# The-Learning-And-Vision-Atelier-LAVA/BUFFER

Measured on AMD Instinct MI355X. Metric: registration pairs/sec, higher is better.
Workload: dtype f32

## Files before the change

buffer_amd/_lib.py:

```python
import ctypes as C
import os

_HERE = os.path.dirname(os.path.abspath(__file__))
LIB_PATH = os.environ.get("BUF_LIB_PATH") or os.path.join(_HERE, "libbuffer_hip.so")

BUF_OK = 0


class BufferHipError(RuntimeError):
    pass


class buf_grid_t(C.Structure):
    _fields_ = [
        ("ws", C.c_void_p), ("ws_bytes", C.c_size_t),
        ("ns", C.c_int), ("nb", C.c_int),
        ("cells_per_elem", C.c_int64),
        ("radius", C.c_float),
        ("supports", C.c_void_p),
        ("desc", C.c_void_p), ("s_off", C.c_void_p), ("table", C.c_void_p),
        ("sorted", C.c_void_p), ("order", C.c_void_p), ("scan_tmp", C.c_void_p),
    ]


class buf_voxel_map_t(C.Structure):
    _fields_ = [
        ("buf", C.c_void_p), ("buf_bytes", C.c_size_t),
        ("nclouds", C.c_int), ("nrows", C.c_int), ("n", C.c_int),
        ("max_cells", C.c_int64),
        ("voxel", C.c_double), ("epsilon", C.c_double),
        ("clouds", C.c_void_p), ("table", C.c_void_p), ("rows", C.c_void_p), ("keys", C.c_void_p), ("row_off", C.c_void_p),
    ]


_lib = None

_vp, _i, _f, _i64, _sz = C.c_void_p, C.c_int, C.c_float, C.c_int64, C.c_size_t

_SIGNATURES = {
    "buf_last_error": (C.c_char_p, []),
    "buf_version": (_i, []),
    "buf_device_count": (_i, []),
    "buf_timing_enable": (None, [_i]),
    "buf_timing_collect": (C.c_longlong, [C.POINTER(C.c_double), C.POINTER(C.c_double)]),
    "buf_timing_collect_kernel": (C.c_longlong, [_i, C.POINTER(C.c_double), C.POINTER(C.c_double)]),
    "buf_grid_default_cells": (_i64, [_i, _i]),
    "buf_grid_ws_bytes": (_sz, [_i, _i, _i64]),
    "buf_grid_cell_dims": (_i, [C.POINTER(C.c_double), _f, _i64, C.POINTER(C.c_double), C.POINTER(C.c_int)]),
    "buf_grid_build": (_i, [C.POINTER(buf_grid_t), _vp, _i, _vp, _i, _f, _i64, _vp, _sz, _vp]),
    "buf_grid_query": (_i, [C.POINTER(buf_grid_t), _vp, _i, _vp, _vp, _f, _i, _vp, _vp, _vp, _vp, _vp]),
    "buf_radius_neighbors": (_i, [_vp, _i, _vp, _i, _vp, _vp, _i, _f, _i, _vp, _vp, _vp, _vp, _sz, _vp]),
    "buf_grid_subsample_ws_bytes": (_sz, [_i, _i, _i64, _i]),
    "buf_grid_subsample_batch": (_i, [_vp, _i, _vp, _i, _f, _i, _vp, _i, _vp, _vp, _vp, _vp, _i64, _vp, _sz, _vp]),
    "buf_fps_ws_bytes": (_sz, [_i, _i]),
    "buf_fps": (_i, [_vp, _i, _i, _i, _vp, _vp, _sz, _vp]),
    "buf_gather": (_i, [_vp, _vp, _i, _i, _i, _i, _vp, _vp]),
    "buf_group": (_i, [_vp, _vp, _i, _i, _i, _i, _i, _vp, _vp]),
    "buf_ball_query": (_i, [_vp, _vp, _i, _i, _i, _f, _i, _vp, _vp]),
    "buf_three_nn": (_i, [_vp, _vp, _i, _i, _i, _vp, _vp, _vp]),
    "buf_select_patches": (_i, [_vp, _vp, _i, _i, _f, _i, _vp, _vp]),
    "buf_select_patches_batched_ws_bytes": (_sz, [_i, _i]),
    "buf_select_patches_batched": (_i, [_vp, _vp, _i, _vp, _i, _f, _i, _vp, _vp, _sz, _vp]),
    "buf_permute_clouds": (_i, [_vp, _vp, _vp, _i, _vp, _vp]),
    "buf_compact_ws_bytes": (_sz, [_i]),
    "buf_compact_greater": (_i, [_vp, _i, _i, _f, _vp, _vp, _vp, _sz, _vp]),
    "buf_knn_ws_bytes": (_sz, [_i, _i, _i]),
    "buf_knn1_ws_bytes": (_sz, [_i, _i, _i]),
    "buf_knn": (_i, [_vp, _vp, _i, _i, _i, _i, _i, _vp, _vp, _vp, _sz, _vp]),
    "buf_fps_ragged": (_i, [_vp, _vp, _i, _i, _vp, _vp, _sz, _vp]),
    "buf_svd3x3_batched": (_i, [_vp, _i, _vp, _vp, _vp, _vp]),
    "buf_vn_gather_block": (_i, [_vp, _vp, _vp, _vp, _i, _i, _i, _i, _i, _i, _f, _vp, _vp, _vp, _vp, _f, _vp, _vp]),
    "buf_vn_gather_pre_supported": (_i, [_i, _i, _i]),
    "buf_vn_gather_pre_ws_bytes": (_sz, [_i, _i]),
    "buf_vn_gather_block_pre": (_i, [_vp, _vp, _vp, _vp, _i, _i, _i, _i, _i, _f, _vp, _vp, _vp, _vp, _f, _vp, _vp, _sz, _vp]),
    "buf_vn_pointwise": (_i, [_vp, _vp, _i, _i, _i, _vp, _i, _i, _i, _vp, _vp, _vp, _vp, _f, _vp, _vp, _vp]),
    "buf_gather_max": (_i, [_vp, _vp, _i, _i, _i, _i, _vp, _vp]),
    "buf_vn_std": (_i, [_vp, _vp, _i, _i, _vp, _vp]),
    "buf_score_head_ws_bytes": (_sz, [_i, _i]),
    "buf_score_head": (_i, [_vp, _i, _vp, _i, _vp, _vp, _vp, _vp, _f, _vp, _vp, _vp, _vp, _f, _vp, _vp, _vp, _vp, _vp, _i, _vp, _vp, _i, _f,
                            _vp, _vp, _sz, _vp]),
    "buf_patch_voxelize_ws_bytes": (_sz, [_i]),
    "buf_patch_voxelize": (_i, [_vp, _vp, _i, _i, _f, _vp, _i, _i, _vp, _f, _i, _vp, _vp, _vp, _vp, _vp, _vp, _vp,
                                _vp, _vp, _sz, _vp]),
    "buf_cylindrical_net_wg": (_i, [_vp, _i, _vp, _vp, _vp, _vp, _vp, _vp, _vp]),
    "buf_cylindrical_net_wg_form": (_i, [_vp, _i, _vp, _vp, _vp, _vp, _vp, _i, _vp, _vp]),
    "buf_cylindrical_net_wg_all": (_i, [_vp, _i, _vp, _vp, _vp, _vp, _vp, _vp, _vp, _vp]),
    "buf_cylindrical_net_wg_all_flags": (_i, [_vp, _vp, _vp, _vp]),
    "buf_cylindrical_net_w25": (_i, [_vp, _i, _vp, _vp, _vp, _vp, _vp, _vp, _vp, _vp, _vp]),
    "buf_cylindrical_net_w25_flags": (_i, [_vp, _vp, _vp, _vp, _vp]),
    "buf_cylindrical_net_split_safe_w25": (_i, [_vp, _i, _vp, _vp, _vp, _vp, _vp, _vp, _vp, _vp, _vp, _vp, _vp, _vp, _vp, _vp]),
    "buf_winograd_f25_tile_weights": (_i, [_vp, _i, _i, _vp]),
    "buf_cylindrical_net_wg_supports": (_i, [_vp, _vp]),
    "buf_cylindrical_net_wg_flags": (_i, [_vp, _vp, _vp]),
    "buf_cylindrical_net_split_safe": (_i, [_vp, _i, _vp, _vp, _vp, _vp, _vp, _vp, _vp, _vp, _vp, _vp, _vp, _vp]),
    "buf_cylindrical_net_split_safe_form": (_i, [_vp, _i, _vp, _vp, _vp, _vp, _vp, _vp, _i, _vp, _vp, _vp, _vp, _vp, _vp]),
    "buf_cost_volume_net_split_safe": (_i, [_vp, _vp, _i, _vp, _vp, _i, _vp, _vp, _vp, _vp, _vp, _vp, _vp, _vp]),
    "buf_cylindrical_net_split_safe_all": (_i, [_vp, _i, _vp, _vp, _vp, _vp, _vp, _vp, _vp, _vp, _vp, _vp, _vp, _vp, _vp]),
    "buf_cylindrical_net_split": (_i, [_vp, _i, _vp, _vp, _vp, _vp, _vp, _vp, _vp, _vp]),
    "buf_cylindrical_net_split_head": (_i, [_vp, _i, _vp, _vp, _vp, _vp, _vp, _vp, _vp, _vp, _vp, _vp]),
    "buf_split_gemm_count": (C.c_longlong, [_i, _i, _i, _i]),
    "buf_split_tile_gemm": (_i, [_vp, _i, _i, _i, _i, _vp]),
    "buf_cost_volume_net_split": (_i, [_vp, _vp, _i, _vp, _vp, _vp, _vp, _vp]),
    "buf_cost_volume_net_split_gather": (_i, [_vp, _i, _vp, _vp, _i, _vp, _vp, _vp, _vp, _vp]),
    "buf_split_filter_count": (C.c_longlong, [_i, _i]),
    "buf_split_tile_filters": (_i, [_vp, _i, _i, _vp]),
    "buf_winograd_tile_weights": (_i, [_vp, _i, _i, _vp]),
    "buf_winograd_f24_tile_weights": (_i, [_vp, _i, _i, _vp]),
    "buf_winograd_group": (_i, [_i, _i]),
    "buf_cost_winograd_group": (_i, [_i]),
    "buf_winograd_tile_filters": (_i, [_vp, _i, _i, _i, _i, _vp]),
    "buf_voxel_downsample_ws_bytes": (_sz, [_i, _i64]),
    "buf_voxel_downsample": (_i, [_vp, _vp, _i, _i, C.c_double, _vp, _vp, _vp, _i64, _vp, _sz, _vp]),
    "buf_voxel_downsample_batch_ws_bytes": (_sz, [_i, _i, _i64]),
    "buf_voxel_downsample_batch": (_i, [_vp, _i, _i, _vp, _i, C.c_double, _vp, _vp, _i64, _vp, _sz, _vp]),
    "buf_knn_normals": (_i, [_vp, _i, _vp, _i, _vp, _i, _i, _vp, _i, _vp, _vp, _vp]),
    "buf_icp_ws_bytes": (_sz, [_i, _i, _i, _i]),
    "buf_icp_batched": (_i, [_vp, _vp, _vp, _vp, _vp, _i, _i, _f, _vp, _i, C.c_double, C.c_double, _vp, _vp, _vp, _vp, _vp,
                             _vp, _sz, _vp]),
    "buf_gicp_batched": (_i, [_vp, _vp, _vp, _vp, _vp, _vp, _i, _f, C.c_double, _vp, _i, C.c_double, C.c_double, _vp, _vp, _vp, _vp,
                              _vp, _vp, _sz, _vp]),
    "buf_pair_stats_ws_bytes": (_sz, [_i, _i, _i, _i, _i64]),
    "buf_pair_stats": (_i, [_vp, _vp, _i, _vp, _vp, _i, _vp, _f, _i64, _vp, _vp, _vp, _vp, _sz, _vp]),
    "buf_pose_graph_ws_bytes": (_sz, [_i, _i, _i, _i]),
    "buf_pose_graph_optimize": (_i, [_vp, _vp, _i, _vp, _vp, _vp, _vp, _vp, _vp, _vp, _vp, _i, C.c_double, C.c_double, C.c_double,
                                     _vp, _vp, _vp, _vp, _vp, _sz, _vp]),
    "buf_fpfh_ws_bytes": (_sz, [_i]),
    "buf_fpfh": (_i, [_vp, _vp, _i, _vp, _i, _i, _vp, _vp, _vp, _sz, _vp]),
    "buf_iss_keypoints": (_i, [_vp, _i, _vp, _i, _vp, _i, _i, C.c_double, C.c_double, _i, _vp, _vp, _vp, _vp]),
    "buf_feature_match_ws_bytes": (_sz, [C.c_longlong, C.c_longlong, _i]),
    "buf_feature_match": (_i, [_vp, _vp, _vp, _vp, _i, _i, _i, _f, _vp, _vp, _vp, _vp, _vp, _sz, _vp]),
    "buf_fgr_ws_bytes": (_sz, [_i, _i, _i]),
    "buf_fgr_batched": (_i, [_vp, _vp, _vp, _vp, _vp, _vp, _i, _vp, C.c_double, _i, _i, C.c_double, C.c_double, _i, C.c_double, _i, _i,
                             _vp, _vp, _vp, _vp, _vp, _sz, _vp]),
    "buf_sc2_ws_bytes": (_sz, [_vp, _i, _i]),
    "buf_sc2_batched": (_i, [_vp, _vp, _vp, _vp, _vp, _vp, _i, C.c_double, C.c_double, C.c_double, _i, _i, C.c_double, _i, _i,
                             _vp, _vp, _vp, _vp, _vp, _vp, _vp, _vp, _sz, _vp]),
    "buf_clique_ws_bytes": (_sz, [_vp, _i, _i, _i]),
    "buf_clique_batched": (_i, [_vp, _vp, _vp, _vp, _vp, _vp, _i, C.c_double, C.c_double, C.c_double, C.c_double, _i, _i, C.c_double, _i,
                                _i, _vp, _vp, _vp, _vp, _vp, _vp, _vp, _vp, _vp, _vp, _vp, _sz, _vp]),
    "buf_voxel_map_bytes": (_sz, [_i, _i, _i64]),
    "buf_voxel_map_ws_bytes": (_sz, [_i, _i, _i64]),
    "buf_voxel_map_build": (_i, [C.POINTER(buf_voxel_map_t), _vp, _vp, _vp, _i, C.c_double, C.c_double, _i64, _vp, _sz, _vp, _sz, _vp]),
    "buf_voxel_map_export": (_i, [C.POINTER(buf_voxel_map_t), _i, _vp, _vp, _vp, _vp, _vp, _vp]),
    "buf_vgicp_ws_bytes": (_sz, [_i, _i]),
    "buf_vgicp_batched": (_i, [C.POINTER(buf_voxel_map_t), _vp, _vp, _vp, _vp, _i, _i, _vp, _i, C.c_double, C.c_double, _vp, _vp, _vp,
                               _vp, _vp, _vp, _sz, _vp]),
    "buf_match_metrics":(_i, [_vp, _vp, _vp, _i, _i, _vp, _vp, _f, _f, _f, _vp, _vp, _vp]),
    "buf_row_linear": (_i, [_vp, _i, _i, _i, _vp, _vp, _i, _vp, _vp]),
    "buf_segment_instance_norm_ws_bytes": (_sz, [_i, _i]),
    "buf_segment_instance_norm": (_i, [_vp, _i, _i, _vp, _i, _f, _vp, _vp, _sz, _vp]),
    "buf_descriptor_head": (_i, [_vp, _i, _vp, _vp, _vp, _vp]),
    "buf_cost_volume_net": (_i, [_vp, _vp, _i, _vp, _vp, _vp, _vp]),
    "buf_cost_volume_net_gather": (_i, [_vp, _i, _vp, _vp, _i, _vp, _vp, _vp, _vp]),
    "buf_cost_volume_net_w24": (_i, [_vp, _vp, _i, _vp, _vp, _vp, _vp, _vp]),
    "buf_cost_volume_net_w24_gather": (_i, [_vp, _i, _vp, _vp, _i, _vp, _vp, _vp, _vp, _vp]),
    "buf_cost_volume_net_split_safe_w24": (_i, [_vp, _vp, _i, _vp, _vp, _i, _vp, _vp, _vp, _vp, _vp, _vp, _vp, _vp, _vp]),
    "buf_cost_volume_net_w24b": (_i, [_vp, _vp, _i, _vp, _vp, _vp, _vp, _vp]),
    "buf_cost_volume_net_w24b_gather": (_i, [_vp, _i, _vp, _vp, _i, _vp, _vp, _vp, _vp, _vp]),
    "buf_cost_volume_net_split_safe_w24b": (_i, [_vp, _vp, _i, _vp, _vp, _i, _vp, _vp, _vp, _vp, _vp, _vp, _vp, _vp, _vp]),
    "buf_hypotheses_score": (_i, [_vp, _vp, _vp, _vp, _vp, _i, _i, _f, _vp, _vp, _vp, _vp, _vp, _vp]),
    "buf_ransac_ws_bytes": (_sz, [_i]),
    "buf_ransac_kabsch": (_i, [_vp, _vp, _vp, _i, _i, C.c_uint64, _f, _f, _vp, _vp, _vp, _sz, _vp]),
    "buf_ransac_masked_ws_bytes": (_sz, [_i, _i]),
    "buf_ransac_kabsch_masked": (_i, [_vp, _vp, _vp, _i, _i, C.c_uint64, _f, _f, _vp, _vp, _vp, _sz, _vp]),
    "buf_post_refine": (_i, [_vp, _vp, _vp, _i, _f, _i, _vp, _vp, _vp]),
    "buf_recover_poses_ws_bytes": (_sz, [_i, _i, _i]),
    "buf_recover_poses_batched": (_i, [_vp, _vp, _vp, _vp, _vp, _vp, _i, _vp, _i, _f, _i, _f, _f, _f, _i, _vp, _vp, _sz, _vp]),
}


def exported_symbols():
    return sorted(_SIGNATURES)


def lib():
    global _lib
    if _lib is None:
        if not os.path.exists(LIB_PATH):
            raise BufferHipError(
                f"{LIB_PATH} is missing: build it with `python -m buffer_amd.build` "
                "(hipcc --offload-arch=gfx950). buffer_amd has no CPU fallback.")
        import torch
        l = C.CDLL(LIB_PATH)
        for name, (res, args) in _SIGNATURES.items():
            fn = getattr(l, name)
            fn.restype = res
            fn.argtypes = args
        _lib = l
    return _lib


def check(rc, what=""):
    if rc != BUF_OK:
        msg = lib().buf_last_error().decode(errors="replace")
        raise BufferHipError(f"{what} failed ({rc}): {msg}")
```

buffer_amd/csrc/buffer_hip.hip:

```cpp
#include <stdlib.h>
#include "core.hip"
#include "radius.hip"
#include "icp.hip"
#include "pairstats.hip"
#include "posegraph.hip"
#include "metrics.hip"
#include "subsample.hip"
#include "pointops.hip"
#include "vn.hip"
#include "voxelize.hip"
#include "registration.hip"
#include "convnet.hip"
#include "convnet_h3.hip"
#include "costnet_h3.hip"
#include "preprocess.hip"
#include "convnet_wg.hip"
#include "convnet_w24.hip"
#include "convnet_w24k.hip"
#include "convnet_w24p.hip"
#include "convnet_w24a.hip"
#include "convnet_w25.hip"
#include "costnet.hip"
#include "costnet_w24.hip"
#include "costnet_w24b.hip"
#include "cnn_launch.hip"
#include "split_safe.hip"
#include "fpfh.hip"
#include "iss.hip"
#include "match.hip"
#include "fgr.hip"
#include "sc2.hip"
#include "clique.hip"
#include "vgicp.hip"
```

buffer_amd/csrc/cnn_launch.hip:

```cpp
#include "common.h"

#define WG_F24_FLAG BUF_CYL_F24
#define BUF_CYL_FORM_LIBRARY BUF_CYL_FORM_PASS_SPLIT
static inline bool wg_f24_flagged(int relu) { return relu >= 2; }

typedef void (*CylKernelFn)(const float*, CylWgParams, float*);
struct CylKernel { CylKernelFn plain, rerun; LdsGrant grant, grant_rerun; };
static CylKernel cyl_wg = { k_cyl_net_wg, k_cyl_net_wg_rerun }, cyl_w24 = { k_cyl_net_w24, k_cyl_net_w24_rerun },
                 cyl_w24k = { k_cyl_net_w24k, k_cyl_net_w24k_rerun }, cyl_w24p = { k_cyl_net_w24p, k_cyl_net_w24p_rerun },
                 cyl_w24a = { k_cyl_net_w24a, k_cyl_net_w24a_rerun }, cyl_w25 = { k_cyl_net_w25, k_cyl_net_w25_rerun };

static CylKernel& cyl_kernel_for(const int* relu, int form, bool sets24, bool sets25)
{
    if (sets25) return cyl_w25;
    if (sets24) return cyl_w24a;
    bool flagged = false, ksplit = false;
    for (int l = 0; l < WG_LAYERS; l++) {
        flagged |= wg_f24_flagged(relu[l]);
        ksplit |= (relu[l] & BUF_CYL_F24K) != 0;
    }
    if (!flagged) return cyl_wg;
    if (!ksplit) return cyl_w24;
    if (form == BUF_CYL_FORM_DEFAULT) form = BUF_CYL_FORM_LIBRARY;
    return form == BUF_CYL_FORM_PASS_SPLIT ? cyl_w24p : cyl_w24k;
}

static int wg_check_widths(const int* cin, const int* cout, bool follow = true)
{
    for (int l = 0; l < WG_LAYERS; l++) {
        const int ci = cin[l], co = cout[l];
        BUF_REQUIRE(ci > 0 && ci % 16 == 0 && ci <= WG_MAXC && (co == 32 || co == 64 || co == 128), BUF_EINVAL,
                    "buf_cylindrical_net_wg: layer %d has unsupported widths %d -> %d", l, ci, co);
        BUF_REQUIRE(co != 128 || ci % 32 == 0, BUF_EINVAL,
                    "buf_cylindrical_net_wg: layer %d has unsupported widths %d -> %d (128 output channels need Cin %% 32 == 0)", l, ci, co);
        BUF_REQUIRE(co != 32 || (ci % 32 == 0 && ci <= 64), BUF_EINVAL,
                    "buf_cylindrical_net_wg: layer %d has unsupported widths %d -> %d (32 output channels need Cin = 32 or 64)", l, ci, co);
        BUF_REQUIRE(l == 0 || ci == cout[l - 1], BUF_EINVAL, "buf_cylindrical_net_wg: layer %d width mismatch", l);
        BUF_REQUIRE(!follow || l == 0 || cout[l - 1] != 32 || co == 32, BUF_EINVAL,
                    "buf_cylindrical_net_wg: layer %d has unsupported widths %d -> %d (only 32-output layers may follow a 32-output layer)", l, ci, co);
    }
    BUF_REQUIRE(cout[WG_LAYERS - 1] == 32, BUF_EINVAL, "buf_cylindrical_net_wg: the last layer must have 32 channels");
    return BUF_OK;
}

static int w24_check_flags(const int* cin, const int* cout, const int* relu)
{
    for (int l = 0; l < WG_LAYERS; l++) {
        BUF_REQUIRE(relu[l] >= 0 && relu[l] <= (BUF_CYL_F24K | WG_F24_FLAG | 1), BUF_EINVAL,
                    "buf_cylindrical_net_wg: layer %d has the relu word %d (bit 0: ReLU, bits 1 and 2: the F(2x4) flags, nothing above)", l, relu[l]);
        BUF_REQUIRE(!(relu[l] & BUF_CYL_F24K) || (cout[l] == 64 && cin[l] % 64 == 0), BUF_EINVAL,
                    "buf_cylindrical_net_wg: the K-split F(2x4) flag (bit 2) goes only on layers with 64 output channels and Cin %% 64 == 0 "
                    "(layer %d: %d -> %d, flags %d)", l, cin[l], cout[l], relu[l]);
        BUF_REQUIRE(((relu[l] & WG_F24_FLAG) != 0) == (cout[l] == 128), BUF_EINVAL,
                    "buf_cylindrical_net_wg: the F(2x4) flag goes on every layer with 128 output channels and on no other (layer %d: %d -> %d, flags %d)",
                    l, cin[l], cout[l], relu[l]);
    }
    return BUF_OK;
}

static int cyl_check(const int* cin, const int* cout, const int* relu, const float* const* wt24_host, const float* const* wt25_host, const char* who)
{
    if (!wt24_host && !wt25_host) {
        if (int rc = wg_check_widths(cin, cout)) return rc;
        for (int l = 0; l < WG_LAYERS; l++)
            if (wg_f24_flagged(relu[l])) return w24_check_flags(cin, cout, relu);
        return BUF_OK;
    }
    for (int l = 0; wt25_host && l < WG_LAYERS; l++)
        BUF_REQUIRE(!wt25_host[l] || ((cout[l] == 64 || cout[l] == 32) && cin[l] > 0 && cin[l] % 16 == 0), BUF_EINVAL,
                    "%s: layer %d (%d -> %d) takes no F(2x5) set (64 or 32 output channels, Cin %% 16 == 0)", who, l, cin[l], cout[l]);
    if (int rc = wg_check_widths(cin, cout, false)) return rc;
    if (int rc = w24_check_flags(cin, cout, relu)) return rc;
    bool f22_ran = false;
    int f22_layer = -1;
    for (int l = 0; l < WG_LAYERS; l++) {
        const bool own24 = wt24_host && wt24_host[l], own25 = wt25_host && wt25_host[l];
        BUF_REQUIRE(!own24 || (!(relu[l] & (WG_F24_FLAG | W24K_FLAG)) && (cout[l] == 64 || cout[l] == 32)), BUF_EINVAL,
                    "%s: layer %d (%d -> %d, flags %d) takes no F(2x4) set of its own (64 or 32 output channels, no F(2x4) flag)",
                    who, l, cin[l], cout[l], relu[l]);
        BUF_REQUIRE(!f22_ran || cout[l] == 32, BUF_EINVAL,
                    "%s: layer %d has unsupported widths %d -> %d (once a 32-output layer in the F(2x2) form has run, layer %d here, "
                    "only 32-output layers may follow)", who, l, cin[l], cout[l], f22_layer);
        if (cout[l] == 32 && !own24 && !own25 && !f22_ran) { f22_ran = true; f22_layer = l; }
    }
    return BUF_OK;
}

extern "C" int buf_cylindrical_net_wg_supports(const int* cin_host, const int* cout_host)
{
    BUF_REQUIRE(cin_host && cout_host, BUF_EINVAL, "buf_cylindrical_net_wg_supports: null argument");
    return wg_check_widths(cin_host, cout_host);
}

extern "C" int buf_cylindrical_net_wg_flags(const int* cin_host, const int* cout_host, const int* relu_host)
{
    BUF_REQUIRE(cin_host && cout_host && relu_host, BUF_EINVAL, "buf_cylindrical_net_wg_flags: null argument");
    return cyl_check(cin_host, cout_host, relu_host, nullptr, nullptr, "buf_cylindrical_net_wg");
}

extern "C" int buf_cylindrical_net_wg_all_flags(const int* cin_host, const int* cout_host, const int* relu_host, const float* const* wt24_host)
{
    BUF_REQUIRE(cin_host && cout_host && relu_host && wt24_host, BUF_EINVAL, "buf_cylindrical_net_wg_all_flags: null argument");
    return cyl_check(cin_host, cout_host, relu_host, wt24_host, nullptr, "buf_cylindrical_net_wg_all");
}

extern "C" int buf_cylindrical_net_w25_flags(const int* cin_host, const int* cout_host, const int* relu_host, const float* const* wt24_host,
                                             const float* const* wt25_host)
{
    BUF_REQUIRE(cin_host && cout_host && relu_host && wt24_host && wt25_host, BUF_EINVAL, "buf_cylindrical_net_w25_flags: null argument");
    return cyl_check(cin_host, cout_host, relu_host, wt24_host, wt25_host, "buf_cylindrical_net_w25");
}

static int cyl_prepare(const float* const* wt_host, const float* const* bias_host, const int* cin_host, const int* cout_host, const int* relu_host,
                       const float* const* wt24_host, const float* const* wt25_host, int form, const char* who, CylWgParams& P, CylKernel*& K)
{
    BUF_REQUIRE(wt_host && bias_host && cin_host && cout_host && relu_host, BUF_EINVAL, "%s: null argument", who);
    for (int l = 0; l < WG_LAYERS; l++) {
        P.wt[l] = wt_host[l]; P.bias[l] = bias_host[l];
        P.cin[l] = cin_host[l]; P.cout[l] = cout_host[l]; P.relu[l] = relu_host[l];
        BUF_REQUIRE(P.wt[l] && P.bias[l], BUF_EINVAL, "%s: null weights for layer %d", who, l);
    }
    if (int rc = cyl_check(P.cin, P.cout, P.relu, wt24_host, wt25_host, who)) return rc;
    P.only_if = nullptr;
    K = &cyl_kernel_for(P.relu, form, wt24_host != nullptr, wt25_host != nullptr);
    if (K == &cyl_wg) return BUF_OK;
    for (int l = 0; l < WG_LAYERS; l++) {
        if (wt25_host && wt25_host[l]) { P.wt[l] = wt25_host[l]; P.relu[l] = (P.relu[l] & 1) | W25_FLAG; }
        else if (P.relu[l] & WG_F24_FLAG) P.wt[l] += W24_SET_F22(P.cin[l]);
        else if (P.relu[l] & W24K_FLAG) P.wt[l] += WG_BLOCKS * P.cout[l] * P.cin[l];
        else if (wt24_host && wt24_host[l]) { P.wt[l] = wt24_host[l]; P.relu[l] |= W24K_FLAG; }
        P.relu[l] &= ~WG_F24_FLAG;
    }
    return BUF_OK;
}

#ifdef WG_STAMP
static int wg_stamp_report(const CylWgParams& P, int npatch, void* stream)
{
    BUF_CHECK_HIP(hipStreamSynchronize((hipStream_t)stream));
    long long* h = (long long*)malloc((size_t)npatch * (4 * 20 + 4) * sizeof(long long));
    BUF_CHECK_HIP(hipMemcpy(h, P.stamps, (size_t)npatch * (4 * 20 + 4) * sizeof(long long), hipMemcpyDeviceToHost));
    double comp[WG_LAYERS][4] = {}, wait[WG_LAYERS][4] = {}, tot = 0, pre = 0; long n = 0;
    for (int b = npatch / 2; b < npatch; b++, n++)
        for (int w = 0; w < 4; w++) {
            const long long* q = h + ((size_t)b * 4 + w) * 20;
            for (int l = 0; l < WG_LAYERS; l++) { comp[l][w] += (double)(q[2 * l + 1] - q[2 * l]); wait[l][w] += (double)(q[2 * l + 2] - q[2 * l + 1]); }
            if (w == 0) { tot += (double)(q[2 * WG_LAYERS] - q[0]); pre += (double)(q[0] - q[17]); }
        }
    if (n && npatch >= 1024) {
        double dc = 0, dr = 0;
        for (int b = npatch / 2; b < npatch; b++) { const long long* q = h + (size_t)npatch * 80 + (size_t)b * 4; dc += (double)(q[2] - q[0]); dr += (double)(q[3] - q[1]); }
        fprintf(stderr, "  WG_STAMP in-kernel clock: %.0f shader cycles per workgroup over %.0f ticks of the 100 MHz counter -> %.3f GHz\n", dc / n, dr / n, dc / dr * 0.1);
        fprintf(stderr, "WG_STAMP: %ld workgroups, layers total %.0f cycles per patch, input phase %.0f\n", n, tot / n, pre / n);
        for (int l = 0; l < WG_LAYERS; l++) {
            const double mf = 38.0 * (P.cin[l] / 4) * (P.cout[l] / 16) / 4;
            fprintf(stderr, "  layer %d %3d->%3d: MFMAs/wave %5.0f | to barrier %7.0f %7.0f %7.0f %7.0f | wait %6.0f %6.0f %6.0f %6.0f | cycles per MFMA slot %.1f\n",
                    l, P.cin[l], P.cout[l], mf, comp[l][0] / n, comp[l][1] / n, comp[l][2] / n, comp[l][3] / n, wait[l][0] / n, wait[l][1] / n,
                    wait[l][2] / n, wait[l][3] / n, (comp[l][0] + wait[l][0]) / n / (2 * mf));
        }
    }
    free(h); (void)hipFree(P.stamps);
    return BUF_OK;
}
#endif

static int cyl_launch(CylKernel& K, const float* x, int npatch, CylWgParams P, float* y, void* stream)
{
    const size_t lds = sizeof(float) * WG_BUF;
    if (int rc = P.only_if ? grant_dynamic_lds((const void*)K.rerun, lds, K.grant_rerun) : grant_dynamic_lds((const void*)K.plain, lds, K.grant)) return rc;
    double macs = 0;
    for (int l = 0; l < WG_LAYERS; l++) macs += 9.0 * P.cin[l] * P.cout[l];
    TimedSpan span;
    bool timed = !P.only_if && timing_begin((hipStream_t)stream, &span, 2.0 * 140 * macs * npatch, BUF_TIMED_CYL_NET);
#ifdef WG_STAMP
    if (&K == &cyl_wg) BUF_CHECK_HIP(hipMalloc(&P.stamps, (size_t)npatch * (4 * 20 + 4) * sizeof(long long)));
#endif
    const CylKernelFn kernel = P.only_if ? K.rerun : K.plain;
    kernel<<<npatch, WG_THREADS, lds, (hipStream_t)stream>>>(x, P, y);
    if (timed) timing_end((hipStream_t)stream, &span);
    BUF_LAUNCH_CHECK();
#ifdef WG_STAMP
    if (&K == &cyl_wg) return wg_stamp_report(P, npatch, stream);
#endif
    return BUF_OK;
}

extern "C" int buf_cylindrical_net_wg_form(const float* x, int npatch, const float* const* wt_host, const float* const* bias_host,
                                           const int* cin_host, const int* cout_host, const int* relu_host, int form, float* y, void* stream)
{
    BUF_REQUIRE(npatch >= 0, BUF_EINVAL, "buf_cylindrical_net_wg: npatch=%d", npatch);
    BUF_REQUIRE(form >= BUF_CYL_FORM_DEFAULT && form <= BUF_CYL_FORM_PASS_SPLIT, BUF_EINVAL,
                "buf_cylindrical_net_wg: form=%d (-1: the library's default, 0: K split, 1: pass split)", form);
    if (npatch == 0) return BUF_OK;
    BUF_REQUIRE(x && y, BUF_EINVAL, "buf_cylindrical_net_wg: null argument");
    CylWgParams P;
    CylKernel* K;
    if (int rc = cyl_prepare(wt_host, bias_host, cin_host, cout_host, relu_host, nullptr, nullptr, form, "buf_cylindrical_net_wg", P, K)) return rc;
    return cyl_launch(*K, x, npatch, P, y, stream);
}

extern "C" int buf_cylindrical_net_wg(const float* x, int npatch, const float* const* wt_host, const float* const* bias_host,
                                      const int* cin_host, const int* cout_host, const int* relu_host, float* y, void* stream)
{
    return buf_cylindrical_net_wg_form(x, npatch, wt_host, bias_host, cin_host, cout_host, relu_host, BUF_CYL_FORM_DEFAULT, y, stream);
}

static int cyl_net_own_sets(const char* who, const float* x, int npatch, const float* const* wt_host, const float* const* bias_host, const int* cin_host,
                            const int* cout_host, const int* relu_host, const float* const* wt24_host, const float* const* wt25_host, bool w25, float* y,
                            void* stream)
{
    BUF_REQUIRE(npatch >= 0, BUF_EINVAL, "%s: npatch=%d", who, npatch);
    if (npatch == 0) return BUF_OK;
    BUF_REQUIRE(x && y && wt24_host && (wt25_host || !w25), BUF_EINVAL, "%s: null argument", who);
    CylWgParams P;
    CylKernel* K;
    if (int rc = cyl_prepare(wt_host, bias_host, cin_host, cout_host, relu_host, wt24_host, wt25_host, BUF_CYL_FORM_DEFAULT, who, P, K)) return rc;
    return cyl_launch(*K, x, npatch, P, y, stream);
}

extern "C" int buf_cylindrical_net_wg_all(const float* x, int npatch, const float* const* wt_host, const float* const* bias_host, const int* cin_host,
                                          const int* cout_host, const int* relu_host, const float* const* wt24_host, float* y, void* stream)
{
    return cyl_net_own_sets("buf_cylindrical_net_wg_all", x, npatch, wt_host, bias_host, cin_host, cout_host, relu_host, wt24_host, nullptr, false, y, stream);
}

extern "C" int buf_cylindrical_net_w25(const float* x, int npatch, const float* const* wt_host, const float* const* bias_host, const int* cin_host,
                                       const int* cout_host, const int* relu_host, const float* const* wt24_host, const float* const* wt25_host, float* y,
                                       void* stream)
{
    return cyl_net_own_sets("buf_cylindrical_net_w25", x, npatch, wt_host, bias_host, cin_host, cout_host, relu_host, wt24_host, wt25_host, true, y, stream);
}

template <typename Q>
struct CostKernel { void (*plain)(const float*, const float*, Q, float*); void (*rerun)(const float*, const float*, Q, float*); const char* name; LdsGrant grant, grant_rerun; };
static CostKernel<CostNetParams> cost_f22 = { k_cost_net, k_cost_net_rerun, "k_cost_net" };
static CostKernel<CostNetW24Params> cost_w24 = { k_cost_net_w24, k_cost_net_w24_rerun, "k_cost_net_w24" };
static CostKernel<CostNetW24BParams> cost_w24b = { k_cost_net_w24b, k_cost_net_w24b_rerun, "k_cost_net_w24b" };

static CostNetParams& cost_net_base(CostNetParams& P) { return P; }
template <typename Q> static CostNetParams& cost_net_base(Q& q) { return q.P; }
static void cost_net_sets(CostNetParams&, const float* const*) {}
template <typename Q> static void cost_net_sets(Q& q, const float* const* f24_host)
{
    for (size_t i = 0; i < sizeof(q.f24) / sizeof(q.f24[0]); i++) q.f24[i] = f24_host[i];
}

template <typename Q>
static int cost_net_prepare(Q& q, const float* const* wt_host, const float* const* bias_host, const float* const* f24_host, const long long* s_rows,
                            const long long* t_rows, int ele_n, const int* only_if, const char* who)
{
    CostNetParams& P = cost_net_base(q);
    for (int l = 0; l < CV_LAYERS; l++) {
        P.wt[l] = wt_host[l]; P.bias[l] = bias_host[l];
        BUF_REQUIRE(P.wt[l] && P.bias[l], BUF_EINVAL, "%s: null weights for layer %d", who, l);
    }
    P.s_rows = s_rows; P.t_rows = t_rows;
    P.chan_floats = s_rows ? ele_n * 20 : 100;
    P.row_floats = 32 * P.chan_floats;
    P.skip_floats = s_rows ? 20 : 0;
    P.only_if = only_if;
    cost_net_sets(q, f24_host);
    return BUF_OK;
}

static const double cost_net_macs_per_match =
    60.0 * 480 * 32 + 54.0 * 288 * 32 + 16.0 * 64 * 96 * 64 +
    16.0 * (49.0 * 64 * 64 + 36.0 * 64 * 128 + 25.0 * 128 * 128 + 16.0 * 128 * 64) +
    36.0 * 576 * 64 + 16.0 * 576 * 32 + 4.0 * 288 * 32 + 1.0 * 128 * 20;

#ifdef CV_STAMP
static int cv_stamp_begin(int m, long long** stamps)
{
    BUF_CHECK_HIP(hipMalloc(stamps, (size_t)m * 16 * sizeof(long long)));
    BUF_CHECK_HIP(hipMemcpyToSymbol(HIP_SYMBOL(cv_stamp_ptr), stamps, sizeof(*stamps)));
    return BUF_OK;
}
static int cv_stamp_end(int m, long long* stamps, void* stream, const char* kernel)
{
    if (m >= 2048) {
        BUF_CHECK_HIP(hipStreamSynchronize((hipStream_t)stream));
        long long* h = (long long*)malloc((size_t)m * 16 * sizeof(long long));
        BUF_CHECK_HIP(hipMemcpy(h, stamps, (size_t)m * 16 * sizeof(long long), hipMemcpyDeviceToHost));
        static const char* name[8] = { "A.1 (layer 0 maps)", "A.2 (layer 1)", "layer 2", "layer 3", "layer 4", "layer 5", "layer 6", "layers 7-9" };
        double d[8] = {};
        for (int b = m / 2; b < m; b++)
            for (int i = 0; i < 8; i++) d[i] += (double)(h[(size_t)b * 16 + i + 1] - h[(size_t)b * 16 + i]);
        for (int i = 0; i < 8; i++) fprintf(stderr, "  CV_STAMP %s %-20s %8.0f cycles per match\n", kernel, name[i], d[i] / (m - m / 2));
        free(h);
    }
    (void)hipFree(stamps);
    return BUF_OK;
}
#endif

template <typename Q>
static int cost_net_launch(CostKernel<Q>& K, const float* s_eq, const float* t_eq, int m, Q q, float* ind_out, void* stream)
{
    const bool rerun = cost_net_base(q).only_if != nullptr;
    size_t lds = sizeof(float) * CV_BUF;
    if (int rc = rerun ? grant_dynamic_lds((const void*)K.rerun, lds, K.grant_rerun) : grant_dynamic_lds((const void*)K.plain, lds, K.grant)) return rc;
    TimedSpan span;
    bool timed = !rerun && timing_begin((hipStream_t)stream, &span, 2.0 * cost_net_macs_per_match * m, BUF_TIMED_COST_NET);
#ifdef CV_STAMP
    long long* stamps = nullptr;
    if (int rc = cv_stamp_begin(m, &stamps)) return rc;
#endif
    const auto kernel = rerun ? K.rerun : K.plain;
    kernel<<<m, CV_THREADS, lds, (hipStream_t)stream>>>(s_eq, t_eq, q, ind_out);
    if (timed) timing_end((hipStream_t)stream, &span);
    BUF_LAUNCH_CHECK();
#ifdef CV_STAMP
    if (int rc = cv_stamp_end(m, stamps, stream, K.name)) return rc;
#endif
    return BUF_OK;
}

template <typename Q>
static int cost_net_run(const char* who, CostKernel<Q>& K, bool gathered, const float* s_eq, const float* t_eq, int ele_n, const long long* s_rows,
                        const long long* t_rows, int m, const float* const* wt_host, const float* const* bias_host, const float* const* f24_host,
                        float* ind_out, void* stream)
{
    if (gathered) BUF_REQUIRE(m >= 0 && ele_n == 7, BUF_EINVAL, "%s: m=%d ele_n=%d (the kernel is built for ele_n = 7)", who, m, ele_n);
    else BUF_REQUIRE(m >= 0, BUF_EINVAL, "%s: m=%d", who, m);
    if (m == 0) return BUF_OK;
    BUF_REQUIRE(s_eq && t_eq && (!gathered || (s_rows && t_rows)) && wt_host && bias_host && (f24_host || std::is_same<Q, CostNetParams>::value) && ind_out,
                BUF_EINVAL, "%s: null argument", who);
    Q q;
    if (int rc = cost_net_prepare(q, wt_host, bias_host, f24_host, s_rows, t_rows, ele_n, nullptr, who)) return rc;
    return cost_net_launch(K, s_eq, t_eq, m, q, ind_out, stream);
}

extern "C" int buf_cost_volume_net(const float* s_eq, const float* t_eq, int m, const float* const* wt_host,
                                   const float* const* bias_host, float* ind_out, void* stream)
{
    return cost_net_run("buf_cost_volume_net", cost_f22, false, s_eq, t_eq, 7, nullptr, nullptr, m, wt_host, bias_host, nullptr, ind_out, stream);
}

extern "C" int buf_cost_volume_net_gather(const float* equi, int ele_n, const long long* s_rows, const long long* t_rows, int m,
                                          const float* const* wt_host, const float* const* bias_host, float* ind_out, void* stream)
{
    return cost_net_run("buf_cost_volume_net_gather", cost_f22, true, equi, equi, ele_n, s_rows, t_rows, m, wt_host, bias_host, nullptr, ind_out, stream);
}

extern "C" int buf_cost_volume_net_w24(const float* s_eq, const float* t_eq, int m, const float* const* wt_host, const float* const* bias_host,
                                       const float* const* f24_host, float* ind_out, void* stream)
{
    return cost_net_run("buf_cost_volume_net_w24", cost_w24, false, s_eq, t_eq, 7, nullptr, nullptr, m, wt_host, bias_host, f24_host, ind_out, stream);
}

extern "C" int buf_cost_volume_net_w24_gather(const float* equi, int ele_n, const long long* s_rows, const long long* t_rows, int m,
                                              const float* const* wt_host, const float* const* bias_host, const float* const* f24_host,
                                              float* ind_out, void* stream)
{
    return cost_net_run("buf_cost_volume_net_w24_gather", cost_w24, true, equi, equi, ele_n, s_rows, t_rows, m, wt_host, bias_host, f24_host, ind_out, stream);
}

extern "C" int buf_cost_volume_net_w24b(const float* s_eq, const float* t_eq, int m, const float* const* wt_host, const float* const* bias_host,
                                        const float* const* f24_host, float* ind_out, void* stream)
{
    return cost_net_run("buf_cost_volume_net_w24b", cost_w24b, false, s_eq, t_eq, 7, nullptr, nullptr, m, wt_host, bias_host, f24_host, ind_out, stream);
}

extern "C" int buf_cost_volume_net_w24b_gather(const float* equi, int ele_n, const long long* s_rows, const long long* t_rows, int m,
                                               const float* const* wt_host, const float* const* bias_host, const float* const* f24_host,
                                               float* ind_out, void* stream)
{
    return cost_net_run("buf_cost_volume_net_w24b_gather", cost_w24b, true, equi, equi, ele_n, s_rows, t_rows, m, wt_host, bias_host, f24_host, ind_out, stream);
}
```

buffer_amd/csrc/convnet_wg.hip:

```cpp
#include "common.h"
#include <type_traits>

#define WG_CS 160
#define WG_ROW 22
#define WG_ZERO 154
#define WG_MAXC 128
#define WG_LAYERS 8
#define WG_THREADS 256
#define WG_BUF (WG_MAXC * WG_CS)
#define WG_KSTEP (16 * WG_CS)
#define WG_BLOCKS 16

typedef float wgf4 __attribute__((ext_vector_type(4)));
typedef float wgf2 __attribute__((ext_vector_type(2)));
typedef const __attribute__((address_space(3))) wgf2* wg_lds_f2;

struct CylWgParams {
    const float* wt[WG_LAYERS];
    const float* bias[WG_LAYERS];
    int cin[WG_LAYERS], cout[WG_LAYERS], relu[WG_LAYERS];
    const int* only_if;
#ifdef WG_STAMP
    long long* stamps;
#endif
};
#ifdef WG_STAMP
#define WG_STAMP_AT(SLOT) if ((threadIdx.x & 63) == 0) P.stamps[((size_t)blockIdx.x * 4 + w) * 20 + (SLOT)] = __builtin_amdgcn_s_memtime();
#else
#define WG_STAMP_AT(SLOT)
#endif

__device__ __forceinline__ bool wg_tile(int t, int idx, int& ty, int& tx)
{
    if (t == 0) { const bool a = idx < 10; ty = a ? 0 : 1; tx = a ? idx : idx - 6; return true; }
    if (t == 1) { const bool a = idx < 10, b = idx < 14; ty = a ? 2 : (b ? 1 : 3); tx = a ? idx : (b ? idx - 10 : idx - 6); return true; }
    ty = 3; tx = 0;
    return false;
}

__device__ __forceinline__ unsigned wg_row_addr(unsigned act_addr, int t, int a, int li, int lk)
{
    if (t == 2) return act_addr + 4u * (unsigned)(lk * WG_CS + (a < 2 ? (5 + a) * WG_ROW + li : WG_ZERO));
    int ty, tx;
    const bool ok = wg_tile(t, li, ty, tx);
    const int row = 2 * ty - 1 + a;
    return act_addr + 4u * (unsigned)(lk * WG_CS + ((ok && row >= 0 && row <= 6) ? row * WG_ROW + 2 * tx : WG_ZERO));
}

__device__ __forceinline__ float wg_add(float a, float b) { float r; asm("v_add_f32 %0, %1, %2" : "=v"(r) : "v"(a), "v"(b)); return r; }
__device__ __forceinline__ float wg_sub(float a, float b) { float r; asm("v_sub_f32 %0, %1, %2" : "=v"(r) : "v"(a), "v"(b)); return r; }

__host__ __device__ constexpr int wg_a1(int I) { return I == 0 ? 0 : 1; }
__host__ __device__ constexpr int wg_a2(int I) { return I == 3 ? 3 : 2; }

__host__ __device__ constexpr bool wg_chains(int I) { return I >= 0 && I < 3; }

#define WG_LOAD2(DST, A0, A1_, OFS)                                                                       \
    {                                                                                                     \
        DST[0] = *(wg_lds_f2)(size_t)((A0) + (OFS));                                                      \
        asm volatile("" : "+v"(A0));                                                                      \
        DST[1] = *(wg_lds_f2)(size_t)((A0) + (OFS) + 8);                                                  \
        asm volatile("" : "+v"(A0));                                                                      \
        DST[2] = *(wg_lds_f2)(size_t)((A1_) + (OFS));                                                     \
        asm volatile("" : "+v"(A1_));                                                                     \
        DST[3] = *(wg_lds_f2)(size_t)((A1_) + (OFS) + 8);                                                 \
        asm volatile("" : "+v"(A1_));                                                                     \
    }


typedef unsigned wgu4 __attribute__((ext_vector_type(4)));
__device__ __forceinline__ __amdgpu_buffer_rsrc_t wg_weights(const float* wt)
{
    return __builtin_amdgcn_make_buffer_rsrc((void*)wt, 0, 0x7fffffff, 0x00027000);
}
__device__ __forceinline__ wgf4 wg_ldw(__amdgpu_buffer_rsrc_t rs, unsigned uniform_float_ofs, unsigned lane_byte_ofs)
{
    return __builtin_bit_cast(wgf4, __builtin_amdgcn_raw_buffer_load_b128(rs, lane_byte_ofs, uniform_float_ofs * 4, 0));
}

template <int I, int NN, int T0, int T1, bool PRIMED, int INEXT, unsigned KSTEP = WG_KSTEP>
__device__ __forceinline__ void wg_pass(unsigned (&RA)[3][4], __amdgpu_buffer_rsrc_t rs, unsigned wp, unsigned wp_next, unsigned lofs, int niter,
                                        int wstride, wgf4 (&W)[NN][2], wgf4 (&acc)[NN][3][4], wgf2 (&D)[2][4])
{
    static_assert(T0 < T1 && T1 <= 2, "the Winograd M-tiles (M-tile 2 is wg_round_direct's)");
    constexpr int A1 = wg_a1(I), A2 = wg_a2(I);
    constexpr int NT = T1 - T0;
    constexpr int A1N = wg_a1(INEXT < 0 ? 0 : INEXT), A2N = wg_a2(INEXT < 0 ? 0 : INEXT);
    float V[2][4];
    unsigned P[NT][2];
#pragma unroll
    for (int t = 0; t < NT; t++) { P[t][0] = RA[T0 + t][A1]; P[t][1] = RA[T0 + t][A2]; }
    if constexpr (!PRIMED) {
#pragma unroll
        for (int g = 0; g < 2; g++) WG_LOAD2(D[g], P[g % NT][0], P[g % NT][1], (g / NT) * KSTEP)
    }
#define WG_XFORM(BUF)                                                                                     \
    {                                                                                                     \
        float r_[4];                                                                                      \
        _Pragma("unroll") for (int b = 0; b < 4; b++) {                                                   \
            const float da_ = D[BUF][b >> 1][b & 1];                                                      \
            const float db_ = D[BUF][2 + (b >> 1)][b & 1];                                                \
            r_[b] = I == 1 ? wg_add(da_, db_) : (I == 2 ? wg_sub(db_, da_) : wg_sub(da_, db_));           \
        }                                                                                                 \
        V[BUF][0] = wg_sub(r_[0], r_[2]); V[BUF][1] = wg_add(r_[1], r_[2]);                               \
        V[BUF][2] = wg_sub(r_[2], r_[1]); V[BUF][3] = wg_sub(r_[1], r_[3]);                               \
    }
    WG_XFORM(0)
#pragma unroll 1
    for (int it = 0; it < niter; it++) {
        const bool more = it + 1 < niter;
        const unsigned wcur = wp + 4 * it * wstride;
        const unsigned wn = more ? wcur + 4 * wstride : wp_next;
        const unsigned adv = more ? 4u * KSTEP : 0u;
        __builtin_amdgcn_sched_barrier(0);
#pragma unroll
        for (int s = 0; s < 4 * NT; s++) {
            const int t = T0 + s % NT, kk = s / NT, g = s + 2;
            if (g < 4 * NT) WG_LOAD2(D[s & 1], P[g % NT][0], P[g % NT][1], (g / NT) * KSTEP)
            else {
                const int t2 = (g - 4 * NT) % NT;
                if ((g - 4 * NT) / NT == 0) { P[t2][0] += adv; P[t2][1] += adv; }
                if constexpr (INEXT >= 0) {
                    unsigned q0 = more ? P[t2][0] : RA[T0 + t2][A1N], q1 = more ? P[t2][1] : RA[T0 + t2][A2N];
                    WG_LOAD2(D[s & 1], q0, q1, ((g - 4 * NT) / NT) * KSTEP)
                } else
                    WG_LOAD2(D[s & 1], P[t2][0], P[t2][1], ((g - 4 * NT) / NT) * KSTEP)
            }
            __builtin_amdgcn_sched_barrier(0);
#pragma unroll
            for (int n = 0; n < NN; n++)
#pragma unroll
                for (int j = 0; j < 4; j++)
                    acc[n][t][j] = __builtin_amdgcn_mfma_f32_16x16x4f32(W[n][kk & 1][j], V[s & 1][j], acc[n][t][j], 0, 0, 0);
            __builtin_amdgcn_sched_barrier(0);
            WG_XFORM((s + 1) & 1)
            if (s % NT == NT - 1) {
#pragma unroll
                for (int n = 0; n < NN; n++)
                    W[n][kk & 1] = kk < 2 ? wg_ldw(rs, wcur + n * 256 + (kk + 2) * wstride, lofs) : wg_ldw(rs, wn + n * 256 + (kk - 2) * wstride, lofs);
            }
            __builtin_amdgcn_sched_barrier(0);
        }
#pragma unroll
        for (int t = 2; t < NT; t++) { P[t][0] += adv; P[t][1] += adv; }
    }
#undef WG_XFORM
}

template <int NN, int T0, int T1, unsigned KSTEP = WG_KSTEP, bool FENCE = false>
__device__ __forceinline__ void wg_round(unsigned (&RA)[3][4], __amdgpu_buffer_rsrc_t rs, unsigned wp, unsigned wp_after, unsigned lofs, int niter,
                                         int wstride, unsigned pstride, const float* __restrict__ bias_lane, wgf4 (&W)[NN][2], wgf4 (&Y)[NN][3][2][2])
{
    using std::integral_constant;
    wgf2 D[2][4];
    wgf4 bv[NN];
#pragma unroll
    for (int n = 0; n < NN; n++) bv[n] = bias_lane ? *reinterpret_cast<const wgf4*>(bias_lane + n * 16) : (wgf4){ 0.f, 0.f, 0.f, 0.f };
    wgf4 acc[NN][3][4];
    float zero = 0.f;
    asm volatile("" : "+v"(zero));
#pragma unroll
    for (int n = 0; n < NN; n++)
#pragma unroll
        for (int t = T0; t < T1; t++)
#pragma unroll
            for (int j = 0; j < 4; j++) acc[n][t][j] = (wgf4){ zero, zero, zero, zero };
    auto run = [&](auto ic) __attribute__((always_inline)) {
        constexpr int I = decltype(ic)::value;
        constexpr int INEXT = I == 3 ? 0 : I + 1;
        if constexpr (I == 1) {
#pragma unroll
            for (int n = 0; n < NN; n++)
#pragma unroll
                for (int t = T0; t < T1; t++) acc[n][t][1] += bv[n];
        }
        constexpr int ICHAIN = (INEXT != 0 && wg_chains(I)) ? INEXT : -1;
        wg_pass<I, NN, T0, T1, wg_chains(I - 1), ICHAIN, KSTEP>(RA, rs, wp + I * pstride, INEXT == 0 ? wp_after : wp + (I + 1) * pstride, lofs, niter, wstride, W, acc, D);
        if constexpr (FENCE) __builtin_amdgcn_sched_barrier(0);
#pragma unroll
        for (int n = 0; n < NN; n++)
#pragma unroll
            for (int t = T0; t < T1; t++) {
                const wgf4 f0 = acc[n][t][0] + acc[n][t][1] + acc[n][t][2];
                const wgf4 f1 = acc[n][t][1] - acc[n][t][2] - acc[n][t][3];
                if constexpr (I == 0) { Y[n][t][1][0] = f0; Y[n][t][1][1] = f1; }
                else if constexpr (I == 1) {
#pragma unroll
                    for (int r = 0; r < 4; r++) {
                        Y[n][t][1][0][r] = __builtin_fmaf(2.f, f0[r], -Y[n][t][1][0][r]);
                        Y[n][t][1][1][r] = __builtin_fmaf(2.f, f1[r], -Y[n][t][1][1][r]);
                    }
                }
                else if constexpr (I == 2) { Y[n][t][0][0] = f0; Y[n][t][0][1] = f1; }
                else { Y[n][t][1][0] -= f0; Y[n][t][1][1] -= f1; }
                if constexpr (I == 2) asm volatile("" : "+v"(Y[n][t][0][0]), "+v"(Y[n][t][0][1]));
                else asm volatile("" : "+v"(Y[n][t][1][0]), "+v"(Y[n][t][1][1]));
            }
    };
    run(integral_constant<int, 0>{});
    run(integral_constant<int, 1>{});
    run(integral_constant<int, 2>{});
    run(integral_constant<int, 3>{});
}

typedef const __attribute__((address_space(3))) float* wg_lds_f1;
#define WG_LOADD(DST, A0, OFS)                                                                            \
    {                                                                                                     \
        _Pragma("unroll") for (int a_ = 0; a_ < 2; a_++)                                                  \
            _Pragma("unroll") for (int b_ = 0; b_ < 3; b_++)                                              \
                DST[a_ * 3 + b_] = *(wg_lds_f1)(size_t)((A0) + (OFS) + 4 * (a_ * WG_ROW + b_));           \
    }
template <int NN>
__device__ __forceinline__ void wg_round_direct(unsigned row5, __amdgpu_buffer_rsrc_t rs, unsigned wp, unsigned lofs, int niter, int wstride,
                                                unsigned pstride, const float* __restrict__ bias_lane, wgf4 (&W)[NN][2], wgf4 (&Y)[NN])
{
    wgf4 Wr[3][NN][2];
#pragma unroll
    for (int n = 0; n < NN; n++)
#pragma unroll
        for (int k = 0; k < 2; k++) {
            Wr[0][n][k] = W[n][k];
            Wr[1][n][k] = wg_ldw(rs, wp + pstride + n * 256 + k * wstride, lofs);
            Wr[2][n][k] = wg_ldw(rs, wp + 2 * pstride + n * 256 + k * wstride, lofs);
        }
    float X[2][6];
    unsigned pa = row5;
    WG_LOADD(X[0], pa, 0)
    WG_LOADD(X[1], pa, WG_KSTEP)
    wgf4 acc[NN][2];
    float zero = 0.f;
    asm volatile("" : "+v"(zero));
#pragma unroll
    for (int n = 0; n < NN; n++) {
        acc[n][0] = bias_lane ? *reinterpret_cast<const wgf4*>(bias_lane + n * 16) : (wgf4){ zero, zero, zero, zero };
        acc[n][1] = (wgf4){ zero, zero, zero, zero };
    }
    float G[NN][6];
#define WG_TAPS(SLOT)                                                                                     \
    _Pragma("unroll") for (int n = 0; n < NN; n++) {                                                      \
        const wgf4 u0_ = Wr[0][n][SLOT], u1_ = Wr[1][n][SLOT], u2_ = Wr[2][n][SLOT];                      \
        const float d1_ = wg_sub(u1_[1], u2_[1]), d2_ = wg_sub(u1_[2], u2_[2]);                           \
        G[n][0] = u0_[0]; G[n][1] = wg_sub(u0_[1], u0_[2]); G[n][2] = u0_[3];                             \
        G[n][3] = wg_sub(u1_[0], u2_[0]); G[n][4] = wg_sub(d1_, d2_); G[n][5] = wg_sub(u1_[3], u2_[3]);   \
    }
#define WG_RELOAD(SLOT, OFS)                                                                              \
    _Pragma("unroll") for (int n = 0; n < NN; n++)                                                        \
        _Pragma("unroll") for (int blk = 0; blk < 3; blk++) Wr[blk][n][SLOT] = wg_ldw(rs, (OFS) + blk * pstride + n * 256, lofs);
    WG_TAPS(0)
    WG_RELOAD(0, wp + 2 * wstride)
#pragma unroll 1
    for (int it = 0; it < niter; it++) {
        const bool more = it + 1 < niter;
        const unsigned wcur = wp + 4 * it * wstride;
        const unsigned wn = more ? wcur + 4 * wstride : wp;
        const unsigned adv = more ? 4u * WG_KSTEP : 0u;
        __builtin_amdgcn_sched_barrier(0);
#pragma unroll
        for (int s = 0; s < 4; s++) {
#pragma unroll
            for (int b = 0; b < 3; b++)
#pragma unroll
                for (int a = 0; a < 2; a++)
#pragma unroll
                    for (int n = 0; n < NN; n++)
                        acc[n][a] = __builtin_amdgcn_mfma_f32_16x16x4f32(G[n][a * 3 + b], X[s & 1][a * 3 + b], acc[n][a], 0, 0, 0);
            __builtin_amdgcn_sched_barrier(0);
            if (s < 2) WG_LOADD(X[s & 1], pa, (s + 2) * WG_KSTEP)
            else {
                if (s == 2) pa += adv;
                WG_LOADD(X[s & 1], pa, (s - 2) * WG_KSTEP)
            }
            __builtin_amdgcn_sched_barrier(0);
            WG_TAPS((s + 1) & 1)
            if (s == 0) WG_RELOAD(1, wcur + 3 * wstride)
            else WG_RELOAD((s + 1) & 1, wn + (s - 1) * wstride)
            __builtin_amdgcn_sched_barrier(0);
        }
    }
#undef WG_TAPS
#undef WG_RELOAD
#pragma unroll
    for (int n = 0; n < NN; n++) Y[n] = acc[n][0] + acc[n][1];
}

template <bool GLB>
__device__ __forceinline__ void wg_store_tile(const wgf4 (&Yt)[2][2], int t, int nt, int relu, float* __restrict__ act, float* __restrict__ out_glb,
                                              int li, int lk)
{
    const int n0 = nt * 16 + lk * 4;
    const float lo = relu ? 0.f : -__builtin_inff();
    {
        int ty, tx;
        const bool valid = wg_tile(t, li, ty, tx);
#pragma unroll
        for (int u = 0; u < 2; u++) {
            const int row = 2 * ty + u;
            const bool ok = valid && row < 7;
            if constexpr (GLB) {
                if (ok) {
#pragma unroll
                    for (int r = 0; r < 4; r++) {
                        const float v0 = fmaxf(Yt[u][0][r], lo), v1 = fmaxf(Yt[u][1][r], lo);
                        *reinterpret_cast<wgf2*>(out_glb + (size_t)(n0 + r) * 140 + row * 20 + 2 * tx) = (wgf2){ v0, v1 };
                    }
                }
            } else {
                const int pos = ok ? row * WG_ROW + 2 * tx + 1 : WG_ZERO + 4;
                const int h0 = (ok && tx == 0) ? row * WG_ROW + 21 : WG_ZERO + 4;
                const int h1 = (ok && tx == 9) ? row * WG_ROW : WG_ZERO + 5;
                float* p = act + n0 * WG_CS;
#pragma unroll
                for (int r = 0; r < 4; r++) {
                    const float v0 = fmaxf(Yt[u][0][r], lo), v1 = fmaxf(Yt[u][1][r], lo);
                    p[r * WG_CS + pos] = v0; p[r * WG_CS + pos + 1] = v1;
                    p[r * WG_CS + h0] = v0; p[r * WG_CS + h1] = v1;
                }
            }
        }
    }
}

template <bool GLB>
__device__ __forceinline__ void wg_store_row6(const wgf4& Yr, int nt, int relu, float* __restrict__ act, float* __restrict__ out_glb, int li, int lk)
{
// ... 296 lines not shown
```

buffer_amd/csrc/split_safe.hip:

```cpp
#include "common.h"


static int cyl_split_safe(const float* x, int npatch, const void* const* wt_split_host, const float* const* bias_host, const int* cin_host,
                          const int* cout_host, const int* relu_host, CylKernel& K, CylWgParams P, const float* head_params, float* y_or_equi,
                          float* desc, int* status_dev, int* flags_ws, void* stream)
{
    hipStream_t s = (hipStream_t)stream;
    BUF_CHECK_HIP(hipMemsetAsync(flags_ws, 0, sizeof(int) * (size_t)npatch, s));
    int relu_split[WG_LAYERS];
    for (int l = 0; l < WG_LAYERS; l++) relu_split[l] = wg_f24_flagged(relu_host[l]) ? (relu_host[l] & 1) : relu_host[l];
    int rc = h3_launch(x, npatch, wt_split_host, bias_host, cin_host, cout_host, relu_split, head_params ? nullptr : y_or_equi, head_params,
                       desc, head_params ? y_or_equi : nullptr, status_dev, stream, flags_ws);
    if (rc) return rc;
    P.only_if = flags_ws;
    rc = cyl_launch(K, x, npatch, P, y_or_equi, stream);
    if (rc) return rc;
    if (head_params) {
        k_desc_head_masked<<<npatch, DH_THREADS, 0, s>>>(y_or_equi, head_params, desc, y_or_equi, flags_ws);
        BUF_LAUNCH_CHECK();
    }
    return BUF_OK;
}

extern "C" int buf_cylindrical_net_split_safe_form(const float* x, int npatch, const void* const* wt_split_host, const float* const* wt_wg_host,
                                                   const float* const* bias_host, const int* cin_host, const int* cout_host, const int* relu_host,
                                                   int form, const float* head_params, float* y_or_equi, float* desc, int* status_dev,
                                                   int* flags_ws, void* stream)
{
    BUF_REQUIRE(npatch >= 0, BUF_EINVAL, "buf_cylindrical_net_split_safe: npatch=%d", npatch);
    if (npatch == 0) return BUF_OK;
    BUF_REQUIRE(x && y_or_equi && flags_ws && wt_split_host && wt_wg_host && bias_host && cin_host && cout_host && relu_host, BUF_EINVAL,
                "buf_cylindrical_net_split_safe: null argument");
    BUF_REQUIRE(!head_params || desc, BUF_EINVAL, "buf_cylindrical_net_split_safe: head without desc");
    BUF_REQUIRE(form >= BUF_CYL_FORM_DEFAULT && form <= BUF_CYL_FORM_PASS_SPLIT, BUF_EINVAL,
                "buf_cylindrical_net_split_safe: form=%d (-1: the library's default, 0: K split, 1: pass split)", form);
    if (int rc = buf_cylindrical_net_wg_flags(cin_host, cout_host, relu_host)) return rc;
    CylWgParams P;
    CylKernel* K;
    if (int rc = cyl_prepare(wt_wg_host, bias_host, cin_host, cout_host, relu_host, nullptr, nullptr, form, "buf_cylindrical_net_wg", P, K)) return rc;
    return cyl_split_safe(x, npatch, wt_split_host, bias_host, cin_host, cout_host, relu_host, *K, P, head_params, y_or_equi, desc, status_dev, flags_ws, stream);
}

extern "C" int buf_cylindrical_net_split_safe(const float* x, int npatch, const void* const* wt_split_host, const float* const* wt_wg_host,
                                              const float* const* bias_host, const int* cin_host, const int* cout_host, const int* relu_host,
                                              const float* head_params, float* y_or_equi, float* desc, int* status_dev, int* flags_ws,
                                              void* stream)
{
    return buf_cylindrical_net_split_safe_form(x, npatch, wt_split_host, wt_wg_host, bias_host, cin_host, cout_host, relu_host, BUF_CYL_FORM_DEFAULT,
                                               head_params, y_or_equi, desc, status_dev, flags_ws, stream);
}

static int cyl_split_safe_own_sets(const char* who, const char* who_f32, const float* x, int npatch, const void* const* wt_split_host,
                                   const float* const* wt_wg_host, const float* const* bias_host, const int* cin_host, const int* cout_host,
                                   const int* relu_host, const float* const* wt24_host, const float* const* wt25_host, bool w25, const float* head_params,
                                   float* y_or_equi, float* desc, int* status_dev, int* flags_ws, void* stream)
{
    BUF_REQUIRE(npatch >= 0, BUF_EINVAL, "%s: npatch=%d", who, npatch);
    if (npatch == 0) return BUF_OK;
    BUF_REQUIRE(x && y_or_equi && flags_ws && wt_split_host, BUF_EINVAL, "%s: null argument", who);
    BUF_REQUIRE(!head_params || desc, BUF_EINVAL, "%s: head without desc", who);
    BUF_REQUIRE(wt24_host && (wt25_host || !w25), BUF_EINVAL, "%s: null argument", who_f32);
    CylWgParams P;
    CylKernel* K;
    if (int rc = cyl_prepare(wt_wg_host, bias_host, cin_host, cout_host, relu_host, wt24_host, wt25_host, BUF_CYL_FORM_DEFAULT, who_f32, P, K)) return rc;
    return cyl_split_safe(x, npatch, wt_split_host, bias_host, cin_host, cout_host, relu_host, *K, P, head_params, y_or_equi, desc, status_dev, flags_ws, stream);
}

extern "C" int buf_cylindrical_net_split_safe_all(const float* x, int npatch, const void* const* wt_split_host, const float* const* wt_wg_host,
                                                  const float* const* bias_host, const int* cin_host, const int* cout_host, const int* relu_host,
                                                  const float* const* wt24_host, const float* head_params, float* y_or_equi, float* desc,
                                                  int* status_dev, int* flags_ws, void* stream)
{
    return cyl_split_safe_own_sets("buf_cylindrical_net_split_safe_all", "buf_cylindrical_net_wg_all", x, npatch, wt_split_host, wt_wg_host, bias_host,
                                   cin_host, cout_host, relu_host, wt24_host, nullptr, false, head_params, y_or_equi, desc, status_dev, flags_ws, stream);
}

extern "C" int buf_cylindrical_net_split_safe_w25(const float* x, int npatch, const void* const* wt_split_host, const float* const* wt_wg_host,
                                                  const float* const* bias_host, const int* cin_host, const int* cout_host, const int* relu_host,
                                                  const float* const* wt24_host, const float* const* wt25_host, const float* head_params,
                                                  float* y_or_equi, float* desc, int* status_dev, int* flags_ws, void* stream)
{
    return cyl_split_safe_own_sets("buf_cylindrical_net_split_safe_w25", "buf_cylindrical_net_w25", x, npatch, wt_split_host, wt_wg_host, bias_host,
                                   cin_host, cout_host, relu_host, wt24_host, wt25_host, true, head_params, y_or_equi, desc, status_dev, flags_ws, stream);
}

template <typename Q>
static int cost_split_safe(const char* who, CostKernel<Q>& K, const float* s_eq, const float* t_eq, int ele_n, const long long* s_rows,
                           const long long* t_rows, int m, const void* const* wt_split_host, const float* const* bias_split_host,
                           const float* const* wt_f32_host, const float* const* bias_f32_host, const float* const* f24_host, float* ind_out,
                           int* status_dev, int* flags_ws, void* stream)
{
    BUF_REQUIRE(m >= 0, BUF_EINVAL, "%s: m=%d", who, m);
    if (m == 0) return BUF_OK;
    BUF_REQUIRE(s_eq && t_eq && wt_split_host && bias_split_host && wt_f32_host && bias_f32_host && (f24_host || std::is_same<Q, CostNetParams>::value) &&
                ind_out && flags_ws, BUF_EINVAL, "%s: null argument", who);
    BUF_REQUIRE((s_rows == nullptr) == (t_rows == nullptr), BUF_EINVAL, "%s: one row list without the other", who);
    BUF_REQUIRE(!s_rows || ele_n == 7, BUF_EINVAL, "%s: ele_n=%d (the kernels are built for ele_n = 7)", who, ele_n);
    Q q;
    if (int rc = cost_net_prepare(q, wt_f32_host, bias_f32_host, f24_host, s_rows, t_rows, ele_n, flags_ws, who)) return rc;
    BUF_CHECK_HIP(hipMemsetAsync(flags_ws, 0, sizeof(int) * (size_t)m, (hipStream_t)stream));
    if (int rc = cost_net_h3_launch(s_eq, t_eq, m, wt_split_host, bias_split_host, s_rows, t_rows, ele_n, ind_out, status_dev, stream, who, flags_ws)) return rc;
    return cost_net_launch(K, s_eq, t_eq, m, q, ind_out, stream);
}

extern "C" int buf_cost_volume_net_split_safe(const float* s_eq, const float* t_eq, int ele_n, const long long* s_rows, const long long* t_rows,
                                              int m, const void* const* wt_split_host, const float* const* bias_split_host,
                                              const float* const* wt_f32_host, const float* const* bias_f32_host, float* ind_out,
                                              int* status_dev, int* flags_ws, void* stream)
{
    return cost_split_safe("buf_cost_volume_net_split_safe", cost_f22, s_eq, t_eq, ele_n, s_rows, t_rows, m, wt_split_host, bias_split_host, wt_f32_host,
                           bias_f32_host, nullptr, ind_out, status_dev, flags_ws, stream);
}

extern "C" int buf_cost_volume_net_split_safe_w24(const float* s_eq, const float* t_eq, int ele_n, const long long* s_rows, const long long* t_rows,
                                                  int m, const void* const* wt_split_host, const float* const* bias_split_host,
                                                  const float* const* wt_f32_host, const float* const* bias_f32_host, const float* const* f24_host,
                                                  float* ind_out, int* status_dev, int* flags_ws, void* stream)
{
    return cost_split_safe("buf_cost_volume_net_split_safe_w24", cost_w24, s_eq, t_eq, ele_n, s_rows, t_rows, m, wt_split_host, bias_split_host, wt_f32_host,
                           bias_f32_host, f24_host, ind_out, status_dev, flags_ws, stream);
}

extern "C" int buf_cost_volume_net_split_safe_w24b(const float* s_eq, const float* t_eq, int ele_n, const long long* s_rows, const long long* t_rows,
                                                   int m, const void* const* wt_split_host, const float* const* bias_split_host,
                                                   const float* const* wt_f32_host, const float* const* bias_f32_host, const float* const* f24_host,
                                                   float* ind_out, int* status_dev, int* flags_ws, void* stream)
{
    return cost_split_safe("buf_cost_volume_net_split_safe_w24b", cost_w24b, s_eq, t_eq, ele_n, s_rows, t_rows, m, wt_split_host, bias_split_host, wt_f32_host,
                           bias_f32_host, f24_host, ind_out, status_dev, flags_ws, stream);
}
```

buffer_amd/ops.py:

```python
import ctypes as C
import time
import os
import numpy as np
import torch

from . import _lib
from ._lib import buf_grid_t, check


def _stream():
    return C.c_void_p(torch.cuda.current_stream().cuda_stream)


def _dev(t, dtype, what):
    if not isinstance(t, torch.Tensor) or not t.is_cuda:
        raise _lib.BufferHipError(f"{what}: expected a tensor in device memory (buffer_amd has no CPU path)")
    if t.dtype != dtype:
        t = t.to(dtype)
    return t.contiguous()


def _ptr(t):
    return C.c_void_p(t.data_ptr()) if t is not None else C.c_void_p(0)

# ... 664 lines not shown
        raise ValueError(f"fgr_batched: {B} pairs but {sd.shape[0]} seeds")
    mt = int(max_tuples)
    T = torch.empty((B, 4, 4), dtype=torch.float64, device=dev)
    info = torch.zeros((B, 4), dtype=torch.int32, device=dev)
    rows = torch.empty((B, 3 * mt, 2), dtype=torch.int32, device=dev) if return_rows else None
    weights = torch.empty((B, 3 * mt), dtype=torch.float64, device=dev) if return_rows else None
    nbytes = max(L.buf_fgr_ws_bytes(int(corr.shape[0]), max(B, 1), mt), 1)
    ws = torch.empty(nbytes, dtype=torch.uint8, device=dev)
    check(L.buf_fgr_batched(_ptr(src), _hptr(sl), _ptr(tgt), _hptr(tl), _ptr(corr), _hptr(cl), B, _hptr(sd), float(tuple_scale), mt,
                            int(trial_factor), float(mu_start), float(delta), int(bool(delta_absolute)), float(division_factor),
                            int(decrease_every), int(iterations), _ptr(T), _ptr(info), _ptr(rows), _ptr(weights), _ptr(ws), nbytes,
                            _stream()), "buf_fgr_batched")
    return T, info, rows, weights


SC2_STATUS = ('NOTHING', 'OK')
SC2_MAX_ROWS, SC2_MAX_SEEDS, SC2_MAX_K1 = 16384, 1024, 128


def sc2_batched(src, src_lengths, tgt, tgt_lengths, corr, corr_lengths, d_thr, inlier_thr, seed_ratio=0.2, max_seeds=512, k1=30,
                nms_radius=0.0, power_iterations=10, refine_iterations=20, return_detail=False):
    L = _lib.lib()
    src, tgt, corr, sl, tl, cl, B, dev = _corr_batch("sc2_batched", src, src_lengths, tgt, tgt_lengths, corr, corr_lengths)
    if B and int(cl.max()) > SC2_MAX_ROWS:
        raise ValueError(f"sc2_batched: {int(cl.max())} correspondences in one pair (at most {SC2_MAX_ROWS})")
    if not (1 <= int(max_seeds) <= SC2_MAX_SEEDS) or not (3 <= int(k1) <= SC2_MAX_K1):
        raise ValueError(f"sc2_batched: max_seeds={max_seeds} (1..{SC2_MAX_SEEDS}), k1={k1} (3..{SC2_MAX_K1})")
    ms, n = int(max_seeds), int(corr.shape[0])
    T = torch.empty((B, 4, 4), dtype=torch.float64, device=dev)
    info = torch.zeros((B, 6), dtype=torch.int32, device=dev)
    detail = None
    if return_detail:
        detail = dict(confidence=torch.empty(n, dtype=torch.float64, device=dev), seeds=torch.empty((B, ms), dtype=torch.int32, device=dev),
                      hyp_counts=torch.empty((B, ms), dtype=torch.int32, device=dev),
                      counts=torch.empty(ms * n, dtype=torch.int32, device=dev), inlier_mask=torch.empty(n, dtype=torch.uint8, device=dev))
    d = detail or {}
    nbytes = max(L.buf_sc2_ws_bytes(_hptr(cl), B, ms), 1) if B else 1
    ws = torch.empty(nbytes, dtype=torch.uint8, device=dev)
    check(L.buf_sc2_batched(_ptr(src), _hptr(sl), _ptr(tgt), _hptr(tl), _ptr(corr), _hptr(cl), B, float(d_thr), float(inlier_thr),
                            float(seed_ratio), ms, int(k1), float(nms_radius), int(power_iterations), int(refine_iterations), _ptr(T),
                            _ptr(info), _ptr(d.get('confidence')), _ptr(d.get('seeds')), _ptr(d.get('hyp_counts')), _ptr(d.get('counts')),
                            _ptr(d.get('inlier_mask')), _ptr(ws), nbytes, _stream()), "buf_sc2_batched")
    return T, info, detail


CLIQUE_STATUS = ('NOTHING', 'OK')
CLIQUE_MAX_SEEDS, CLIQUE_MAX_MEMBERS = 1024, 512


def clique_batched(src, src_lengths, tgt, tgt_lengths, corr, corr_lengths, d_thr, tim_thr=None, t_thr=None, inlier_thr=None,
                   max_seeds=64, max_members=256, gnc_factor=1.4, gnc_iterations=100, refine_iterations=20, return_detail=False):
    L = _lib.lib()
    src, tgt, corr, sl, tl, cl, B, dev = _corr_batch("clique_batched", src, src_lengths, tgt, tgt_lengths, corr, corr_lengths)
    if B and int(cl.max()) > SC2_MAX_ROWS:
        raise ValueError(f"clique_batched: {int(cl.max())} correspondences in one pair (at most {SC2_MAX_ROWS})")
    if not (1 <= int(max_seeds) <= CLIQUE_MAX_SEEDS) or not (3 <= int(max_members) <= CLIQUE_MAX_MEMBERS):
        raise ValueError(f"clique_batched: max_seeds={max_seeds} (1..{CLIQUE_MAX_SEEDS}), max_members={max_members} "
                         f"(3..{CLIQUE_MAX_MEMBERS})")
    d_thr = float(d_thr)
    tim_thr = d_thr if tim_thr is None else float(tim_thr)
    t_thr = d_thr / 2 if t_thr is None else float(t_thr)
    inlier_thr = d_thr if inlier_thr is None else float(inlier_thr)
    ms, mm, n = int(max_seeds), int(max_members), int(corr.shape[0])
    T = torch.empty((B, 4, 4), dtype=torch.float64, device=dev)
    info = torch.zeros((B, 8), dtype=torch.int32, device=dev)
    detail = None
    if return_detail:
        i32 = lambda *shape: torch.empty(shape, dtype=torch.int32, device=dev)
        detail = dict(deg=i32(n), core=i32(n), rank=i32(n), sizes=i32(B, ms), members=i32(B, mm),
                      weights=torch.empty((B, mm * (mm - 1) // 2), dtype=torch.float64, device=dev),
                      pose0=torch.empty((B, 12), dtype=torch.float64, device=dev), inlier_mask=torch.empty(n, dtype=torch.uint8, device=dev))
    d = detail or {}
    nbytes = max(L.buf_clique_ws_bytes(_hptr(cl), B, ms, mm), 1) if B else 1
    ws = torch.empty(nbytes, dtype=torch.uint8, device=dev)
    check(L.buf_clique_batched(_ptr(src), _hptr(sl), _ptr(tgt), _hptr(tl), _ptr(corr), _hptr(cl), B, d_thr, tim_thr, t_thr, inlier_thr, ms,
                               mm, float(gnc_factor), int(gnc_iterations), int(refine_iterations), _ptr(T), _ptr(info), _ptr(d.get('deg')),
                               _ptr(d.get('core')), _ptr(d.get('rank')), _ptr(d.get('sizes')), _ptr(d.get('members')),
                               _ptr(d.get('weights')), _ptr(d.get('pose0')), _ptr(d.get('inlier_mask')), _ptr(ws), nbytes, _stream()),
          "buf_clique_batched")
    return T, info, detail


def pair_stats(points, lengths, pair_src, pair_tgt, T, radius, correspondences=False, cells_per_elem=0):
    L = _lib.lib()
    points = _dev(points, torch.float32, "pair_stats.points")
    if points.dim() != 2 or points.shape[1] != 3:
        raise ValueError(f"pair_stats: points {tuple(points.shape)} is not [N,3]")
    ln, pa, pb = _host_i32(lengths), _host_i32(pair_src), _host_i32(pair_tgt)
    if pa.shape != pb.shape:
        raise ValueError(f"pair_stats: {pa.shape[0]} sources but {pb.shape[0]} targets")
    if int(ln.sum()) != int(points.shape[0]):
        raise ValueError(f"pair_stats: lengths sum to {int(ln.sum())}, points holds {int(points.shape[0])} rows")
    Cn, P, dev = int(ln.shape[0]), int(pa.shape[0]), points.device
    T = _dev(T, torch.float64, "pair_stats.T").reshape(P, 4, 4)
    ok = (pa >= 0) & (pa < Cn)
    rows = int(ln[pa[ok]].astype(np.int64).sum())
    matched = torch.zeros((P,), dtype=torch.int32, device=dev)
    moments = torch.zeros((P, 10), dtype=torch.float64, device=dev)
    nn = torch.empty((max(rows, 1),), dtype=torch.int32, device=dev) if correspondences else None
    nbytes = max(L.buf_pair_stats_ws_bytes(int(points.shape[0]), max(Cn, 1), max(P, 1), rows, int(cells_per_elem)), 1)
    ws = torch.empty(nbytes, dtype=torch.uint8, device=dev)
    check(L.buf_pair_stats(_ptr(points), _hptr(ln), Cn, _hptr(pa), _hptr(pb), P, _ptr(T), float(radius), int(cells_per_elem),
                           _ptr(matched), _ptr(moments), _ptr(nn), _ptr(ws), nbytes, _stream()), "buf_pair_stats")
    return matched, moments, (nn[:rows] if nn is not None else None)


PG_MAX_NODES = 128
PG_STATUS = ('NOTHING', 'CONVERGED_STEP', 'CONVERGED_COST', 'MAX_ITER', 'STALLED', 'FAILED')
PG_TICK_HZ = 1e8


def pose_graph_optimize(nodes, edges, edge_i, edge_j, Z, info, uncertain, fixed, mu, X_init, max_iterations=100, eps_step=1e-9,
                        eps_cost=1e-10, tau0=1e-5, want_ticks=False):
    L = _lib.lib()
    nd, ed, fx = _host_i32(nodes), _host_i32(edges), _host_i32(fixed)
    ei, ej = _host_i32(edge_i), _host_i32(edge_j)
    un = np.ascontiguousarray(uncertain, dtype=np.uint8).reshape(-1)
    mu = np.ascontiguousarray(mu, dtype=np.float64).reshape(-1)
    G = int(nd.shape[0])
    if not (ed.shape[0] == G and fx.shape[0] == G and mu.shape[0] == G):
        raise ValueError(f"pose_graph_optimize: {G} graphs but {ed.shape[0]} edge counts, {fx.shape[0]} fixed nodes, {mu.shape[0]} weights")
    if (nd < 0).any() or (ed < 0).any():
        raise ValueError("pose_graph_optimize: negative node or edge count")
    N, E = int(nd.astype(np.int64).sum()), int(ed.astype(np.int64).sum())
    if not (ei.shape[0] == E and ej.shape[0] == E and un.shape[0] == E):
        raise ValueError(f"pose_graph_optimize: {E} edges but {ei.shape[0]} / {ej.shape[0]} node ids, {un.shape[0]} flags")
    X_init = _dev(X_init, torch.float64, "pose_graph_optimize.X_init").reshape(N, 4, 4)
    dev = X_init.device
    Z = _dev(Z, torch.float64, "pose_graph_optimize.Z").reshape(E, 4, 4)
    info = _dev(info, torch.float64, "pose_graph_optimize.info").reshape(E, 6, 6)
    X = torch.empty((N, 4, 4), dtype=torch.float64, device=dev)
    status = torch.zeros((G, 3), dtype=torch.int32, device=dev)
    cost = torch.zeros((G, 2), dtype=torch.float64, device=dev)
    edge = torch.zeros((E, 2), dtype=torch.float64, device=dev)
    nbytes = max(L.buf_pose_graph_ws_bytes(max(G, 1), N, E, min(int(nd.max()) if G else 0, PG_MAX_NODES)), 1)
    ws = torch.zeros(nbytes, dtype=torch.uint8, device=dev)
    check(L.buf_pose_graph_optimize(_hptr(nd), _hptr(ed), G, _hptr(ei), _hptr(ej), _ptr(Z), _ptr(info), _hptr(un), _hptr(fx), _hptr(mu),
                                    _ptr(X_init), int(max_iterations), float(eps_step), float(eps_cost), float(tau0), _ptr(X), _ptr(status),
                                    _ptr(cost), _ptr(edge), _ptr(ws), nbytes, _stream()), "buf_pose_graph_optimize")
    if want_ticks:
        return X, status, cost, edge, ws[:32 * G].view(torch.int64).reshape(G, 4).clone()
    return X, status, cost, edge


METRIC_COLUMNS = ('rep_src', 'rep_tgt', 'nn_inl', 'mutual', 'mutual_inl', 'cons', 'cons_true')


def match_metrics(kp, s_nn, t_nn, T_gt, T_est, tau_kp, tau_match, dist_th, want_d2=False):
    L = _lib.lib()
    kp = _dev(kp, torch.float32, "match_metrics.kp")
    s_nn, t_nn = _dev(s_nn, torch.int32, "match_metrics.s_nn"), _dev(t_nn, torch.int32, "match_metrics.t_nn")
    if s_nn.dim() != 2 or s_nn.shape != t_nn.shape:
        raise ValueError(f"match_metrics: s_nn {tuple(s_nn.shape)} and t_nn {tuple(t_nn.shape)} must both be [B,P]")
    B, P = int(s_nn.shape[0]), int(s_nn.shape[1])
    if kp.dim() != 2 or tuple(kp.shape) != (2 * B * P, 3):
        raise ValueError(f"match_metrics: kp {tuple(kp.shape)} is not [2*{B}*{P},3]")
    dev = kp.device
    T_gt = torch.as_tensor(T_gt, dtype=torch.float64).to(dev).reshape(B, 4, 4).contiguous()
    T_est = _dev(T_est, torch.float32, "match_metrics.T_est").reshape(B, 4, 4).contiguous()
    counts = torch.empty((B, len(METRIC_COLUMNS)), dtype=torch.int32, device=dev)
    d2 = torch.empty((2 * B * P,), dtype=torch.float32, device=dev) if want_d2 else None
    check(L.buf_match_metrics(_ptr(kp), _ptr(s_nn), _ptr(t_nn), B, P, _ptr(T_gt), _ptr(T_est), float(tau_kp), float(tau_match),
                              float(dist_th), _ptr(counts), _ptr(d2), _stream()), "buf_match_metrics")
    return (counts, d2) if want_d2 else counts


def recover_poses_batched(ind, ss_kpts, tt_kpts, ss_R, tt_R, seg_lengths, seeds, cfg):
    L = _lib.lib()
    seg = _host_i32(seg_lengths)
    nb, M = int(seg.shape[0]), int(seg.sum())
    dev = ss_kpts.device
    poses = torch.empty((nb, 4, 4), dtype=torch.float32, device=dev)
    if nb == 0:
        return poses
    nbytes = L.buf_recover_poses_ws_bytes(M, nb, int(cfg.ransac_hypotheses))
    ws = torch.empty(nbytes, dtype=torch.uint8, device=dev)
    sd = (C.c_ulonglong * nb)(*[int(x) & _MASK64 for x in seeds])
    check(L.buf_recover_poses_batched(_ptr(ind.contiguous()), _ptr(ss_kpts.contiguous()), _ptr(tt_kpts.contiguous()),
                                      _ptr(ss_R.contiguous()), _ptr(tt_R.contiguous()), _hptr(seg), nb, sd, int(cfg.azi_n),
                                      float(cfg.inlier_th), int(cfg.ransac_hypotheses), float(cfg.dist_th), float(cfg.similar_th),
                                      float(cfg.refine_threshold), 20 if cfg.pose_refine else 0, _ptr(poses), _ptr(ws), nbytes,
                                      _stream()), "buf_recover_poses_batched")
    return poses


def mfma_tile_weights(wt, lk_major=False):
    K, cout = wt.shape
    assert K % 16 == 0 and cout % 16 == 0
    t = wt.reshape(K // 16, 4, 4, cout // 16, 16)
    perm = (0, 3, 1, 4, 2) if lk_major else (0, 3, 2, 4, 1)
    return np.ascontiguousarray(np.transpose(t, perm), dtype=np.float32).reshape(-1)


def winograd_tile_weights(w, ng=None, blocks=4):
    cout, cin = w.shape[0], w.shape[1]
    assert cin % 4 == 0 and cout % 16 == 0
    if ng is None:
        ng = _lib.lib().buf_winograd_group(cin, cout)
    G = np.array([[1, 0, 0], [.5, .5, .5], [.5, -.5, .5], [0, 0, 1]], np.float64)
    G5 = np.concatenate([G, [[0, 1, 0]]])
    U = np.einsum('ia,ocab,jb->ijoc', G5, np.asarray(w, np.float64), G)
    U = U[:blocks].reshape(blocks, 4, cout // (16 * ng), ng, 16, cin // 4, 4)
    return np.ascontiguousarray(np.transpose(U, (2, 0, 5, 3, 6, 4, 1)), dtype=np.float32).reshape(-1)


def winograd_f24_tile_weights(w):
    cout, cin = w.shape[0], w.shape[1]
    assert cin % 4 == 0 and cout % 32 == 0
    U = winograd_f24_filters(w)
    U = U.reshape(4, 6, cout // 32, 2, 16, cin // 4, 4)
    U = np.transpose(U, (2, 0, 5, 3, 6, 4, 1))
    lead = U.shape[:3]
    wide = U[..., [0, 1, 2, 5]].reshape(*lead, 512)
    narrow = U[..., [3, 4]].reshape(*lead, 256)
    return np.ascontiguousarray(np.concatenate([wide, narrow], axis=-1), dtype=np.float32).reshape(-1)


F24_G2 = np.array([[1, 0, 0], [.5, .5, .5], [.5, -.5, .5], [0, 0, 1]], np.float64)
F24_G4 = np.array([[.25, 0, 0], [-1 / 6, -1 / 6, -1 / 6], [-1 / 6, 1 / 6, -1 / 6], [1 / 24, 1 / 12, 1 / 6], [1 / 24, -1 / 12, 1 / 6], [0, 0, 1]],
                  np.float64)


def winograd_f24_filters(w):
    w64 = np.asarray(w, np.float64)
    U = np.zeros((4, 6) + w64.shape[:2], np.float64)
    for a in range(3):
        for b in range(3):
            U += (F24_G2[:, a][:, None, None, None] * w64[None, None, :, :, a, b]) * F24_G4[:, b][None, :, None, None]
    return U


F25_POINTS = (0.0, 1.0, -1.0, 2.0, -2.0, 0.5, -0.5)


def _f25_matrices():
    pts = np.array(F25_POINTS, np.float64)
    bt = np.zeros((7, 7))
    g = np.zeros((7, 3))
    for j, p in enumerate(pts):
        lj = np.poly(np.delete(pts, j))[::-1]
        bt[j] = lj
        nj = np.prod(p - np.delete(pts, j))
        g[j] = [1 / nj, p / nj, p * p / nj]
    at = pts[None, :] ** np.arange(5)[:, None]
    return np.round(bt * 16) / 16, g, at


F25_B5T, F25_G5, F25_A5T = _f25_matrices()


def winograd_f25_filters(w):
    w64 = np.asarray(w, np.float64)
    U = np.zeros((4, 7) + w64.shape[:2], np.float64)
    for a in range(3):
        for b in range(3):
            U += (F24_G2[:, a][:, None, None, None] * w64[None, None, :, :, a, b]) * F25_G5[:, b][None, :, None, None]
    return U


def winograd_f25_tile_weights(w):
    cout, cin = w.shape[0], w.shape[1]
    assert cin % 4 == 0 and cout % 16 == 0
    U = winograd_f25_filters(w).reshape(4, 7, cout // 16, 16, cin // 4, 4)
    U = np.transpose(U, (0, 4, 2, 5, 3, 1))
    lead = U.shape[:3]
    parts = [U[..., 0:4].reshape(*lead, 256), U[..., 4:6].reshape(*lead, 128), U[..., 6:7].reshape(*lead, 64)]
    return np.ascontiguousarray(np.concatenate(parts, axis=-1), dtype=np.float32).reshape(-1)


F24_FLAG = 2
F24K_FLAG = 4
F24P_DEFAULT = True
F24A_DEFAULT = 'all'
F24A_PARTS = {'all': (64, 32), 'out64': (64,), 'out32': (32,), 'off': (), None: ()}


F25_DEFAULT = 'out64'
F25_PARTS = {'all': (64, 32), 'out64': (64,), 'out32': (32,), 'off': (), None: ()}


def form_parts(name, value, default, table):
    value = default if value is None else 'all' if value is True else 'off' if value is False else value
    if value not in table:
        raise ValueError(f"{name} = {value!r}: one of " + ", ".join(repr(k) for k in table if k is not None))
    return table[value]


def cyl_f25_parts(f24, f24k, f24p, f25):
    explicit = not (f24 is None and f24k is None and f24p is None)
    if f25 == 'out128':
        raise ValueError("f25 = 'out128': the 128-output layers have no F(2x5) form (csrc/convnet_w25.hip)")
    parts = form_parts('f25', f25, None if explicit else F25_DEFAULT, F25_PARTS)
    if parts and explicit and not (f24 in (None, True) and f24k in (None, True) and f24p in (None, True)):
        raise ValueError("f25 goes with the default forms of the other layers (f24, f24k, f24p left alone or true)")
    return parts


def cyl_f25_filters(layers, parts, device):
    sets = [torch.from_numpy(winograd_f25_tile_weights(w)).to(device)
            if (w.shape[0] in parts and w.shape[0] in (32, 64) and w.shape[1] % 16 == 0) else None for w, _, _ in layers]
    return sets, (C.c_void_p * len(sets))(*[None if t is None else t.data_ptr() for t in sets])


def cyl_layer_filters(w, f24k=True):
    wt = winograd_tile_weights(w)
    cout, cin = w.shape[0], w.shape[1]
    if cout == 128:
        flag = F24_FLAG
    elif f24k and cout == 64 and cin % 64 == 0:
        flag = F24K_FLAG
    else:
        return wt, 0
    return np.concatenate([wt, winograd_f24_tile_weights(w)]), flag


def cyl_f24a_parts(f24, f24k, f24p, f24a):
    explicit = not (f24 is None and f24k is None and f24p is None)
    f24, f24k, f24p = (True if f24 is None else f24), (True if f24k is None else f24k), (F24P_DEFAULT if f24p is None else f24p)
    parts = form_parts('f24a', f24a, None if explicit else F24A_DEFAULT, F24A_PARTS)
    if parts and not (f24 and f24k and f24p):
        raise ValueError("f24a goes with the default forms of the other layers (f24, f24k, f24p left alone or true)")
    return f24, f24k, f24p, parts


def cyl_f24a_filters(layers, flags, parts, device):
    sets = [torch.from_numpy(winograd_f24_tile_weights(w)).to(device)
            if (flag == 0 and w.shape[0] in parts and w.shape[0] in (32, 64) and w.shape[1] % 16 == 0) else None
            for (w, _, _), flag in zip(layers, flags)]
    return sets, (C.c_void_p * len(sets))(*[None if t is None else t.data_ptr() for t in sets])


class CylindricalNet:

    def __init__(self, layers, device, f24=None, f24k=None, f24p=None, f24a=None, f25=None):
        parts25 = cyl_f25_parts(f24, f24k, f24p, f25)
        f24, f24k, f24p, parts = cyl_f24a_parts(f24, f24k, f24p, f24a)
        self.wt, self.bias, self.cin, self.cout, self.relu = [], [], [], [], []
        self.entry = "buf_cylindrical_net_wg"
        self.form = 1 if f24p else 0
        flags = []
        for w, b, relu in layers:
            cout, cin = w.shape[0], w.shape[1]
            wt, flag = cyl_layer_filters(w, f24k) if f24 else (winograd_tile_weights(w), 0)
            flags.append(flag)
            self.wt.append(torch.from_numpy(wt).to(device))
            self.bias.append(torch.from_numpy(np.ascontiguousarray(b, dtype=np.float32)).to(device))
            self.cin.append(cin); self.cout.append(cout); self.relu.append(1 if relu else 0)
        n = len(layers)
        self._wp = (C.c_void_p * n)(*[t.data_ptr() for t in self.wt])
        self._bp = (C.c_void_p * n)(*[t.data_ptr() for t in self.bias])
        self._ci = (C.c_int * n)(*self.cin)
        self._co = (C.c_int * n)(*self.cout)
        self._re = (C.c_int * n)(*[r | f for r, f in zip(self.relu, flags)])
        self.wt24, self._w24p = cyl_f24a_filters(layers, flags, parts, device)
        self.f24_layers = [l for l, t in enumerate(self.wt24) if t is not None]
        self.f24_all = bool(self.f24_layers) and all(f or t is not None for f, t in zip(flags, self.wt24))
        self.wt25, self._w25p = cyl_f25_filters(layers, parts25, device)
        self.f25_layers = [l for l, t in enumerate(self.wt25) if t is not None]
        if self.f25_layers:
            fn, safe, self._extra = "w25", "split_safe_w25", (self._w24p, self._w25p)
        elif self.f24_layers:
            fn, safe, self._extra = "wg_all", "split_safe_all", (self._w24p,)
        else:
            fn, safe, self._extra = "wg_form", "split_safe_form", (self.form,)
        self.fn, self.fn_split_safe = "buf_cylindrical_net_" + fn, "buf_cylindrical_net_" + safe

    def __call__(self, x):
        x = x.contiguous()
        P = x.shape[0]
        y = torch.empty((P, self.cout[-1], 7, 20), dtype=torch.float32, device=x.device)
        check(getattr(_lib.lib(), self.fn)(_ptr(x), P, self._wp, self._bp, self._ci, self._co, self._re, *self._extra, _ptr(y), _stream()), self.fn)
        return y


def split_tile_filters(w):
    L = _lib.lib()
    w = np.ascontiguousarray(w, dtype=np.float32)
    cout, cin = w.shape[0], w.shape[1]
    out = np.empty(L.buf_split_filter_count(cout, cin), dtype=np.uint16)
    check(L.buf_split_tile_filters(w.ctypes.data, cout, cin, out.ctypes.data), "buf_split_tile_filters")
    return out


class CylindricalNetSplit:

    def __init__(self, layers, device, f24k=None, f24p=None, f24a=None, f25=None):
        cyl_f25_parts(None, f24k, f24p, f25)
        form = cyl_f24a_parts(None, f24k, f24p, f24a)[2]
        self.wt, self.bias, self.cin, self.cout, self.relu = [], [], [], [], []
        self.entry = "buf_cylindrical_net_split"
        self.f24_layers, self.f24_all, self.f25_layers = [], False, []
        self.form = 1 if form else 0
        for w, b, relu in layers:
            cout, cin = w.shape[0], w.shape[1]
            self.wt.append(torch.from_numpy(split_tile_filters(w).view(np.int16)).to(device))
            self.bias.append(torch.from_numpy(np.ascontiguousarray(b, dtype=np.float32)).to(device))
            self.cin.append(cin); self.cout.append(cout); self.relu.append(1 if relu else 0)
        n = len(layers)
        self.status = torch.zeros(1, dtype=torch.int32, device=device)
        self._wp = (C.c_void_p * n)(*[t.data_ptr() for t in self.wt])
        self._bp = (C.c_void_p * n)(*[t.data_ptr() for t in self.bias])
        self._ci = (C.c_int * n)(*self.cin)
        self._co = (C.c_int * n)(*self.cout)
        self._re = (C.c_int * n)(*self.relu)
        self.last_flags = None
        self.safe = n == 8 and _lib.lib().buf_cylindrical_net_wg_supports(self._ci, self._co) == 0 and not os.environ.get('BUF_SPLIT_UNSAFE')
        self.f32 = CylindricalNet(layers, device, f24k=f24k, f24p=f24p, f24a=f24a, f25=f25) if self.safe else None
        if self.safe:
            f = self.f32
            self.wt_wg, self._wwp, self._re_safe = f.wt, f._wp, f._re
            self.wt24, self._w24p, self.f24_layers, self.f24_all = f.wt24, f._w24p, f.f24_layers, f.f24_all
            self.wt25, self._w25p, self.f25_layers = f.wt25, f._w25p, f.f25_layers
            self.fn = f.fn_split_safe

    def _safe_call(self, x, head):
        x = x.contiguous()
        P = x.shape[0]
        out = torch.empty((P, self.cout[-1], 7, 20), dtype=torch.float32, device=x.device)
        desc = torch.empty((P, 32), dtype=torch.float32, device=x.device) if head is not None else None
        self.last_flags = torch.empty((max(P, 1),), dtype=torch.int32, device=x.device)
        check(getattr(_lib.lib(), self.fn)(_ptr(x), P, self._wp, self._wwp, self._bp, self._ci, self._co, self._re_safe, *self.f32._extra,
                                           _ptr(head.params) if head is not None else None, _ptr(out), _ptr(desc), _ptr(self.status),
                                           _ptr(self.last_flags), _stream()), self.fn)
        return (desc, out) if head is not None else out

    def __call__(self, x):
        if self.safe:
            return self._safe_call(x, None)
        L = _lib.lib()
        x = x.contiguous()
        P = x.shape[0]
        y = torch.empty((P, self.cout[-1], 7, 20), dtype=torch.float32, device=x.device)
        check(L.buf_cylindrical_net_split(_ptr(x), P, self._wp, self._bp, self._ci, self._co, self._re, _ptr(y), _ptr(self.status), _stream()),
              self.entry)
        return y

    def with_head(self, x, head):
        if self.safe:
            return self._safe_call(x, head)
        L = _lib.lib()
        x = x.contiguous()
        P = x.shape[0]
        desc = torch.empty((P, 32), dtype=torch.float32, device=x.device)
        equi = torch.empty((P, 32, 7, 20), dtype=torch.float32, device=x.device)
        check(L.buf_cylindrical_net_split_head(_ptr(x), P, self._wp, self._bp, self._ci, self._co, self._re, _ptr(head.params),
                                               _ptr(desc), _ptr(equi), _ptr(self.status), _stream()), "buf_cylindrical_net_split_head")
        return desc, equi

    def range_fallbacks(self):
        return 0 if self.last_flags is None else int((self.last_flags != 0).sum().item())

    def check_range(self):
        if int(self.status.item()) != 0:
            self.status.zero_()
            if not self.safe:
                raise FloatingPointError("buf_cylindrical_net_split: an activation left the f16 range (|v| >= 65504); use the fp32 kernel")


class DescriptorHead:

    def __init__(self, w0, b0, w3, b3, device):
        f = lambda a, n: np.asarray(a, dtype=np.float32).reshape(n)
        self.params = torch.from_numpy(np.concatenate([f(w0, 512), f(b0, 16), f(w3, 16), f(b3, 1)])).to(device)

    def __call__(self, y):
        L = _lib.lib()
        y = y.contiguous()
        P = y.shape[0]
        assert y.dtype == torch.float32 and y.numel() == P * 32 * 140
        desc = torch.empty((P, 32), dtype=torch.float32, device=y.device)
        equi = torch.empty((P, 32, 7, 20), dtype=torch.float32, device=y.device)
        check(L.buf_descriptor_head(_ptr(y), P, _ptr(self.params), _ptr(desc), _ptr(equi), _stream()), "buf_descriptor_head")
        return desc, equi


def split_tile_gemm(w, nt):
    L = _lib.lib()
    w = np.ascontiguousarray(w, dtype=np.float32)
    cout, cin, ntaps = w.shape
    out = np.empty(L.buf_split_gemm_count(cout, cin, ntaps, nt), dtype=np.uint16)
    check(L.buf_split_tile_gemm(w.ctypes.data, cout, cin, ntaps, nt, out.ctypes.data), "buf_split_tile_gemm")
    return out


def separate_cost_layer0(w):
    w = np.asarray(w, np.float64)
    cout, cin = w.shape[0], w.shape[1]
    ws = np.zeros((3, 5, cin, cout))
    for dn in range(3):
        for dl in range(3):
            ws[:, dl - dn + 2] += np.transpose(w[:, :, dn, :, dl], (2, 1, 0))
    wt = np.transpose(w.sum(2), (2, 3, 1, 0))
    return ws.reshape(-1, cout).astype(np.float32), wt.reshape(-1, cout).astype(np.float32)


COST_F24_DEFAULT = 'all'
COST_F24_PARTS = {'all': (2, 4, 6), 'l2': (2,), 'l4': (4,), 'l6': (6,), 'off': (), None: ()}


def cost_f24_parts(f24):
    return form_parts('f24', f24, COST_F24_DEFAULT, COST_F24_PARTS)


def cost_f24_filters(layers, parts):
    sets = []
    for l in (2, 4, 6):
        if l not in parts:
            sets.append(None)
            continue
        w = layers[l][0]
        assert tuple(w.shape[2:]) == (3, 1, 3), w.shape
        w2d = np.ascontiguousarray(w[:, :, :, 0, :])
        sets.append(winograd_tile_weights(w2d, ng=1) if l == 6 else winograd_f24_tile_weights(w2d))
    return sets


COST_F24B_DEFAULT = 'all'
COST_F24B_PARTS = {'all': (1, 3), 'l1': (1,), 'l3': (3,), 'off': ()}


def cost_f24b_parts(f24, f24b):
    return form_parts('f24b', f24b, COST_F24B_DEFAULT if f24 is None else 'off', COST_F24B_PARTS)


def cost_f24b_filters(layers, parts):
    sets = []
    for l in (1, 3):
        if l not in parts:
            sets.append(None)
            continue
        w = layers[l][0]
        if l == 1:
            assert tuple(w.shape) == (64, 32, 3, 3, 3), w.shape
            w2d = np.ascontiguousarray(np.transpose(w, (0, 3, 1, 2, 4)).reshape(64, 96, 3, 3))
        else:
            assert tuple(w.shape[2:]) == (3, 1, 3), w.shape
            w2d = np.ascontiguousarray(w[:, :, :, 0, :])
        sets.append(winograd_f24_tile_weights(w2d))
    return sets


class CostVolumeNet:

    def __init__(self, layers, device, f24=None, f24b=None):
        assert len(layers) == 10
        self.parts = cost_f24_parts(f24)
        self.parts_b = cost_f24b_parts(f24, f24b)
        self.wt24 = [None if a is None else torch.from_numpy(a).to(device) for a in cost_f24_filters(layers, self.parts)]
        self._fp = (C.c_void_p * 3)(*[None if t is None else t.data_ptr() for t in self.wt24])
        self.wt24b = [None if a is None else torch.from_numpy(a).to(device) for a in cost_f24b_filters(layers, self.parts_b)]
        self._fpb = (C.c_void_p * 5)(*[None if t is None else t.data_ptr() for t in self.wt24 + self.wt24b])
        self.wt, self.bias = [], []
        for i, (w, b) in enumerate(layers):
            cout, cin = w.shape[0], w.shape[1]
            b = np.asarray(b, np.float32)
            if i == 0:
                assert tuple(w.shape) == (32, 32, 3, 3, 3), w.shape
                tiled = np.concatenate([mfma_tile_weights(m, lk_major=True) for m in separate_cost_layer0(w)])
                self.wt.append(torch.from_numpy(tiled).to(device))
                self.bias.append(torch.from_numpy(np.ascontiguousarray(b)).to(device))
                continue
            if i == 1:
                assert tuple(w.shape) == (64, 32, 3, 3, 3), w.shape
                w2d = np.ascontiguousarray(np.transpose(w, (0, 3, 1, 2, 4)).reshape(64, 96, 3, 3))
                self.wt.append(torch.from_numpy(winograd_tile_weights(w2d, ng=_lib.lib().buf_cost_winograd_group(1))).to(device))
                self.bias.append(torch.from_numpy(np.ascontiguousarray(b)).to(device))
                continue
            if 2 <= i <= 5:
                assert tuple(w.shape[2:]) == (3, 1, 3), w.shape
                tiled = winograd_tile_weights(np.ascontiguousarray(w[:, :, :, 0, :]), ng=_lib.lib().buf_cost_winograd_group(i))
                self.wt.append(torch.from_numpy(tiled).to(device))
                self.bias.append(torch.from_numpy(np.ascontiguousarray(b)).to(device))
                continue
            wt = np.transpose(w, (2, 3, 4, 1, 0)).reshape(-1, cout)
            if i == 9:
                wt = np.concatenate([wt, np.zeros((wt.shape[0], 32 - cout), np.float32)], 1)
                b = np.concatenate([b, np.zeros(32 - cout, np.float32)])
            self.wt.append(torch.from_numpy(mfma_tile_weights(np.ascontiguousarray(wt, dtype=np.float32), lk_major=True)).to(device))
            self.bias.append(torch.from_numpy(np.ascontiguousarray(b)).to(device))
        self._wp = (C.c_void_p * 10)(*[t.data_ptr() for t in self.wt])
        self._bp = (C.c_void_p * 10)(*[t.data_ptr() for t in self.bias])
        if self.parts_b:
            self.kernel, self._sets = "_w24b", (self._fpb,)
        elif self.parts:
            self.kernel, self._sets = "_w24", (self._fp,)
        else:
            self.kernel, self._sets = "", ()

    def _run(self, s_eq, t_eq, s_rows, t_rows, m):
        out = torch.empty((m,), dtype=torch.float32, device=s_eq.device)
        fn = "buf_cost_volume_net" + self.kernel + ("" if s_rows is None else "_gather")
        head = (_ptr(s_eq), _ptr(t_eq), m) if s_rows is None else (_ptr(s_eq), 7, _ptr(s_rows), _ptr(t_rows), m)
        check(getattr(_lib.lib(), fn)(*head, self._wp, self._bp, *self._sets, _ptr(out), _stream()), fn)
        return out

    def __call__(self, s_eq, t_eq):
        s_eq, t_eq = s_eq.contiguous(), t_eq.contiguous()
        return self._run(s_eq, t_eq, None, None, s_eq.shape[0])

    def gathered(self, equi, s_rows, t_rows):
        equi = _dev(equi, torch.float32, "CostVolumeNet.gathered")
        if equi.dim() != 4 or tuple(equi.shape[1:]) != (32, 7, 20):
            raise _lib.BufferHipError(f"CostVolumeNet.gathered: expected [rows,32,7,20] maps, got {tuple(equi.shape)}")
        s_rows, t_rows = _dev(s_rows, torch.int64, "s_rows"), _dev(t_rows, torch.int64, "t_rows")
        return self._run(equi, equi, s_rows, t_rows, int(s_rows.shape[0]))


class CostVolumeNetSplit:

    def __init__(self, layers, device, f24=None, f24b=None):
        assert len(layers) == 10
        self.parts = cost_f24_parts(f24)
        self.parts_b = cost_f24b_parts(f24, f24b)
        mats = []
        w0 = layers[0][0]
        assert tuple(w0.shape) == (32, 32, 3, 3, 3), w0.shape
        ws, wt = separate_cost_layer0(w0)
        mats.append((np.transpose(ws.reshape(15, 32, 32), (2, 1, 0)), 2))
        mats.append((np.transpose(wt.reshape(9, 32, 32), (2, 1, 0)), 2))
        w1 = layers[1][0]
        assert tuple(w1.shape) == (64, 32, 3, 3, 3), w1.shape
        mats.append((np.transpose(w1, (0, 3, 1, 2, 4)).reshape(64, 96, 9), 2))
        for i in range(2, 9):
            w = layers[i][0]
            assert tuple(w.shape[2:]) == (3, 1, 3), w.shape
            mats.append((np.ascontiguousarray(w[:, :, :, 0, :]).reshape(w.shape[0], w.shape[1], 9), 2 if i < 7 else 1))
        w9 = layers[9][0]
        assert tuple(w9.shape) == (20, 32, 2, 1, 2), w9.shape
        mats.append((np.ascontiguousarray(w9[:, :, :, 0, :]).reshape(20, 32, 4), 1))
        self.wt = [torch.from_numpy(split_tile_gemm(m, nt).view(np.int16)).to(device) for m, nt in mats]
        self.bias = []
        for i, (_, b) in enumerate(layers):
            b = np.asarray(b, np.float32)
            if i == 9:
                b = np.concatenate([b, np.zeros(32 - b.shape[0], np.float32)])
            self.bias.append(torch.from_numpy(np.ascontiguousarray(b)).to(device))
        self.status = torch.zeros(1, dtype=torch.int32, device=device)
        self._wp = (C.c_void_p * 11)(*[t.data_ptr() for t in self.wt])
        self._bp = (C.c_void_p * 10)(*[t.data_ptr() for t in self.bias])
        self.safe = not os.environ.get('BUF_SPLIT_UNSAFE')
        self.f32 = CostVolumeNet(layers, device, f24=f24, f24b=f24b) if self.safe else None
        self.last_flags = None

    def _safe(self, s_eq, t_eq, s_rows, t_rows, m, dev):
        out = torch.empty((m,), dtype=torch.float32, device=dev)
        self.last_flags = torch.empty((max(m, 1),), dtype=torch.int32, device=dev)
        fn = "buf_cost_volume_net_split_safe" + self.f32.kernel
        check(getattr(_lib.lib(), fn)(_ptr(s_eq), _ptr(t_eq), 7, _ptr(s_rows), _ptr(t_rows), m, self._wp, self._bp, self.f32._wp, self.f32._bp,
                                      *self.f32._sets, _ptr(out), _ptr(self.status), _ptr(self.last_flags), _stream()), fn)
        return out

    def __call__(self, s_eq, t_eq):
        L = _lib.lib()
        s_eq, t_eq = s_eq.contiguous(), t_eq.contiguous()
        m = s_eq.shape[0]
        if self.safe:
            return self._safe(s_eq, t_eq, None, None, m, s_eq.device)
        out = torch.empty((m,), dtype=torch.float32, device=s_eq.device)
        check(L.buf_cost_volume_net_split(_ptr(s_eq), _ptr(t_eq), m, self._wp, self._bp, _ptr(out), _ptr(self.status), _stream()),
              "buf_cost_volume_net_split")
        return out

    def gathered(self, equi, s_rows, t_rows):
        L = _lib.lib()
        equi = _dev(equi, torch.float32, "CostVolumeNetSplit.gathered")
        if equi.dim() != 4 or tuple(equi.shape[1:]) != (32, 7, 20):
            raise _lib.BufferHipError(f"CostVolumeNetSplit.gathered: expected [rows,32,7,20] maps, got {tuple(equi.shape)}")
        s_rows, t_rows = _dev(s_rows, torch.int64, "s_rows"), _dev(t_rows, torch.int64, "t_rows")
        m = int(s_rows.shape[0])
        if self.safe:
            return self._safe(equi, equi, s_rows, t_rows, m, equi.device)
        out = torch.empty((m,), dtype=torch.float32, device=equi.device)
        check(L.buf_cost_volume_net_split_gather(_ptr(equi), 7, _ptr(s_rows), _ptr(t_rows), m, self._wp, self._bp, _ptr(out),
                                                 _ptr(self.status), _stream()), "buf_cost_volume_net_split_gather")
        return out

    def range_fallbacks(self):
        return 0 if self.last_flags is None else int((self.last_flags != 0).sum().item())

    def check_range(self):
        if int(self.status.item()) != 0:
            self.status.zero_()
            if not self.safe:
                raise FloatingPointError("buf_cost_volume_net_split: a value left the f16 range (|v| >= 65504); use the fp32 kernel")
```

include/buffer_hip.h:

```cpp
#ifndef BUFFER_HIP_H
#define BUFFER_HIP_H
#include <stddef.h>
#include <stdint.h>
#ifdef __cplusplus
extern "C" {
#endif

#define BUF_OK            0
#define BUF_EINVAL       -1
#define BUF_EHIP         -2
#define BUF_EWORKSPACE   -3
#define BUF_ECAPACITY    -4
#define BUF_ENODEVICE    -5

const char* buf_last_error(void);
int         buf_version(void);
int         buf_device_count(void);
#define BUF_TIMED_GRID_QUERY 0
#define BUF_TIMED_CYL_NET    1
#define BUF_TIMED_COST_NET   2
#define BUF_TIMED_SELECT_PATCHES 3
#define BUF_TIMED_PATCH_VOXELIZE 4
#define BUF_TIMED_FPS            5
#define BUF_TIMED_NN1            6
#define BUF_TIMED_VN_GATHER      7
#define BUF_TIMED_GRID_SUBSAMPLE 8
#define BUF_TIMED_DESC_HEAD      9
#define BUF_TIMED_CYL_NET_SPLIT  10
#define BUF_TIMED_COST_NET_SPLIT 11
#define BUF_TIMED_SPFH           12
#define BUF_TIMED_FPFH           13
#define BUF_TIMED_SC2_COMPAT     14
#define BUF_TIMED_SC2_CONF       15
#define BUF_TIMED_SC2_COUNTS     16
#define BUF_TIMED_SC2_HYP        17
#define BUF_TIMED_SC2_REFINE     18
#define BUF_TIMED_CLIQUE_GRAPH   19
#define BUF_TIMED_CLIQUE_PEEL    20
#define BUF_TIMED_CLIQUE_ORDER   21
#define BUF_TIMED_CLIQUE_WALK    22
#define BUF_TIMED_CLIQUE_POSE    23
#define BUF_TIMED_CLIQUE_POLISH  24
#define BUF_TIMED_ISS_SALIENCY   25
#define BUF_TIMED_ISS_NMS        26
#define BUF_TIMED_NKERNELS       27
void        buf_timing_enable(int on);
long long   buf_timing_collect(double* total_ms, double* total_bytes);
long long   buf_timing_collect_kernel(int kernel_id, double* total_ms, double* total_work);

typedef struct buf_grid {
    void*   ws;
    size_t  ws_bytes;
    int     ns, nb;
    int64_t cells_per_elem;
    float   radius;
    const float* supports;
    void*   desc;
    int*    s_off;
    int*    table;
    void*   sorted;
    int*    order;
    void*   scan_tmp;
} buf_grid_t;

int64_t buf_grid_default_cells(int ns, int nb);
size_t  buf_grid_ws_bytes(int ns, int nb, int64_t cells_per_elem);
int     buf_grid_cell_dims(const double* ext, float radius, int64_t cells_per_elem, double* edge_out, int* dim_out);
int     buf_grid_build(buf_grid_t* g, const float* supports, int ns, const int* s_batches_host, int nb,
                       float radius, int64_t cells_per_elem, void* ws, size_t ws_bytes, void* stream);
int     buf_grid_query(const buf_grid_t* g, const float* queries, int nq, const int* q_batches_host,
                       const int* q_order, float radius, int k_out, int* nbr_out, int* counts_out,
                       int* max_count_out, void* todo_ws, void* stream);
int     buf_radius_neighbors(const float* queries, int nq, const float* supports, int ns,
                             const int* q_batches_host, const int* s_batches_host, int nb, float radius,
                             int k_out, int* nbr_out, int* counts_out, int* max_count_out,
                             void* ws, size_t ws_bytes, void* stream);

size_t  buf_grid_subsample_ws_bytes(int n, int nb, int64_t max_cells, int fdim);
int     buf_grid_subsample_batch(const float* pts, int n, const int* batches_host, int nb, float dl,
                                 int max_p, const float* feats, int fdim, float* out_pts, float* out_feats,
                                 int* out_batches_host, int* out_m_host,
                                 int64_t max_cells, void* ws, size_t ws_bytes, void* stream);

size_t  buf_fps_ws_bytes(int b, int n);
int     buf_fps(const float* xyz, int b, int n, int m, int* idx_out, void* ws, size_t ws_bytes, void* stream);
int     buf_fps_ragged(const float* xyz, const int* lengths_host, int b, int m, int* idx_out, void* ws, size_t ws_bytes,
                       void* stream);
int     buf_gather(const float* feat, const int* idx, int b, int c, int n, int m, float* out, void* stream);
int     buf_group(const float* feat, const int* idx, int b, int c, int n, int m, int nsample, float* out, void* stream);
int     buf_ball_query(const float* xyz, const float* new_xyz, int b, int n, int m, float radius, int nsample,
                       int* idx, void* stream);
int     buf_three_nn(const float* unknown, const float* known, int b, int n, int m, float* dist, int* idx, void* stream);
int     buf_select_patches(const float* pts, const float* kpts, int n, int m, float radius, int nsample,
                           float* patches, void* stream);
size_t  buf_select_patches_batched_ws_bytes(int n_total, int nc);
int     buf_select_patches_batched(const float* pts, const int* lengths_host, int nc, const float* kpts, int m, float radius,
                                   int nsample, float* patches, void* ws, size_t ws_bytes, void* stream);
int     buf_permute_clouds(const float* const* clouds_host, const int* lengths_host, const unsigned long long* keys_host,
                           int nc, float* out, void* stream);

size_t  buf_compact_ws_bytes(int n);
int     buf_compact_greater(const float* x, int stride, int n, float threshold, int* idx_out, int* count_out,
                            void* ws, size_t ws_bytes, void* stream);

size_t  buf_knn_ws_bytes(int b, int q, int k);
size_t  buf_knn1_ws_bytes(int b, int n, int q);
int     buf_knn(const float* ref, const float* query, int b, int n, int q, int d, int k, float* dist,
                long long* idx, void* ws, size_t ws_bytes, void* stream);

int     buf_svd3x3_batched(const float* a, int n, float* u, float* s, float* v, void* stream);

int     buf_vn_gather_block(const float* q_pts, const float* s_pts, const float* feats, const int* idx,
                            int nq, int ns, int k, int cin, int cout, int mode, float scale,
                            const float* wf, const float* wd, const float* bn_scale, const float* bn_shift,
                            float slope, float* out, void* stream);
int     buf_vn_gather_pre_supported(int k, int cin, int cout);
size_t  buf_vn_gather_pre_ws_bytes(int ns, int cout);
int     buf_vn_gather_block_pre(const float* q_pts, const float* s_pts, const float* feats, const int* idx,
                                int nq, int ns, int k, int cin, int cout, float scale,
                                const float* wf, const float* wd, const float* bn_scale, const float* bn_shift,
                                float slope, float* out, void* ws, size_t ws_bytes, void* stream);
int     buf_vn_pointwise(const float* a, const int* ind_a, int ind_stride, int na, int ca, const float* b, int cb,
                         int n, int cout, const float* wf, const float* wd, const float* bn_scale,
                         const float* bn_shift, float slope, const float* residual, float* out, void* stream);
int     buf_gather_max(const float* feats, const int* idx, int nq, int ns, int k, int width, float* out, void* stream);
int     buf_row_linear(const float* x, int n, int cin, int cout, const float* w, const float* b, int activation, float* out,
                       void* stream);
size_t  buf_segment_instance_norm_ws_bytes(int nseg, int c);
int     buf_segment_instance_norm(const float* x, int n, int c, const int* lens_host, int nseg, float eps, float* out,
                                  void* ws, size_t ws_bytes, void* stream);
int     buf_vn_std(const float* x, const float* z, int n, int c, float* out, void* stream);
size_t  buf_score_head_ws_bytes(int n, int nseg);
int     buf_score_head(const float* x, int n, const int* lens_host, int nseg,
                       const float* vn1_wf, const float* vn1_wd, const float* vn1_bsc, const float* vn1_bsh, float vn1_slope,
                       const float* vn2_wf, const float* vn2_wd, const float* vn2_bsc, const float* vn2_bsh, float vn2_slope,
                       const float* lin, const float* w0, const float* b0, const float* w1, const float* b1, int c1,
                       const float* w2, const float* b2, int final_activation, float eps, float* out,
                       void* ws, size_t ws_bytes, void* stream);

size_t  buf_patch_voxelize_ws_bytes(int ncentres);
int     buf_patch_voxelize(const float* patches, const float* axis, int npatch, int npts, float des_r,
                           const float* centres, int ncentres, int azi_n, const float* azi_cs, float voxel_r,
                           int nsample, const float* mlp_w_host, const float* mlp_b_host, const float* bn_scale_host,
                           const float* bn_shift_host, float* out_x, float* out_R, float* out_rand, float* out_patches,
                           void* ws, size_t ws_bytes, void* stream);

int     buf_winograd_group(int cin, int cout);
int     buf_winograd_tile_weights(const float* w_host, int cout, int cin, float* out_host);
int     buf_winograd_tile_filters(const float* w_host, int cout, int cin, int ng, int nblk, float* out_host);
#define BUF_CYL_F24 2
#define BUF_CYL_F24K 4
int     buf_cylindrical_net_wg_flags(const int* cin_host, const int* cout_host, const int* relu_host);
int     buf_winograd_f24_tile_weights(const float* w_host, int cout, int cin, float* out_host);
int     buf_cylindrical_net_wg(const float* x, int npatch, const float* const* wt_host, const float* const* bias_host,
                               const int* cin_host, const int* cout_host, const int* relu_host, float* y, void* stream);
#define BUF_CYL_FORM_DEFAULT (-1)
#define BUF_CYL_FORM_K_SPLIT 0
#define BUF_CYL_FORM_PASS_SPLIT 1
int     buf_cylindrical_net_wg_form(const float* x, int npatch, const float* const* wt_host, const float* const* bias_host,
                                    const int* cin_host, const int* cout_host, const int* relu_host, int form, float* y, void* stream);
int     buf_cylindrical_net_wg_supports(const int* cin_host, const int* cout_host);
int     buf_cylindrical_net_wg_all_flags(const int* cin_host, const int* cout_host, const int* relu_host, const float* const* wt24_host);
int     buf_cylindrical_net_wg_all(const float* x, int npatch, const float* const* wt_host, const float* const* bias_host,
                                   const int* cin_host, const int* cout_host, const int* relu_host, const float* const* wt24_host,
                                   float* y, void* stream);
int     buf_winograd_f25_tile_weights(const float* w_host, int cout, int cin, float* out_host);
int     buf_cylindrical_net_w25_flags(const int* cin_host, const int* cout_host, const int* relu_host, const float* const* wt24_host,
                                      const float* const* wt25_host);
int     buf_cylindrical_net_w25(const float* x, int npatch, const float* const* wt_host, const float* const* bias_host,
                                const int* cin_host, const int* cout_host, const int* relu_host, const float* const* wt24_host,
                                const float* const* wt25_host, float* y, void* stream);

long long buf_split_filter_count(int cout, int cin);
int     buf_split_tile_filters(const float* w_host, int cout, int cin, unsigned short* out_host);
int     buf_cylindrical_net_split(const float* x, int npatch, const void* const* wt_host, const float* const* bias_host,
                                  const int* cin_host, const int* cout_host, const int* relu_host, float* y, int* status_dev, void* stream);
int     buf_cylindrical_net_split_head(const float* x, int npatch, const void* const* wt_host, const float* const* bias_host,
                                       const int* cin_host, const int* cout_host, const int* relu_host, const float* head_params,
                                       float* desc, float* equi, int* status_dev, void* stream);

int     buf_cylindrical_net_split_safe(const float* x, int npatch, const void* const* wt_split_host, const float* const* wt_wg_host,
                                       const float* const* bias_host, const int* cin_host, const int* cout_host, const int* relu_host,
                                       const float* head_params, float* y_or_equi, float* desc, int* status_dev, int* flags_ws, void* stream);

int     buf_cylindrical_net_split_safe_form(const float* x, int npatch, const void* const* wt_split_host, const float* const* wt_wg_host,
                                            const float* const* bias_host, const int* cin_host, const int* cout_host, const int* relu_host,
                                            int form, const float* head_params, float* y_or_equi, float* desc, int* status_dev, int* flags_ws,
                                            void* stream);
int     buf_cylindrical_net_split_safe_all(const float* x, int npatch, const void* const* wt_split_host, const float* const* wt_wg_host,
                                           const float* const* bias_host, const int* cin_host, const int* cout_host, const int* relu_host,
                                           const float* const* wt24_host, const float* head_params, float* y_or_equi, float* desc,
                                           int* status_dev, int* flags_ws, void* stream);
int     buf_cylindrical_net_split_safe_w25(const float* x, int npatch, const void* const* wt_split_host, const float* const* wt_wg_host,
                                           const float* const* bias_host, const int* cin_host, const int* cout_host, const int* relu_host,
                                           const float* const* wt24_host, const float* const* wt25_host, const float* head_params,
                                           float* y_or_equi, float* desc, int* status_dev, int* flags_ws, void* stream);

int     buf_descriptor_head(const float* y, int npatch, const float* params, float* desc, float* equi, void* stream);

int     buf_cost_winograd_group(int layer);
int     buf_cost_volume_net(const float* s_eq, const float* t_eq, int m, const float* const* wt_host,
                            const float* const* bias_host, float* ind_out, void* stream);
int     buf_cost_volume_net_gather(const float* equi, int ele_n, const long long* s_rows, const long long* t_rows, int m,
                                   const float* const* wt_host, const float* const* bias_host, float* ind_out, void* stream);
int     buf_cost_volume_net_w24(const float* s_eq, const float* t_eq, int m, const float* const* wt_host, const float* const* bias_host,
                                const float* const* f24_host, float* ind_out, void* stream);
int     buf_cost_volume_net_w24_gather(const float* equi, int ele_n, const long long* s_rows, const long long* t_rows, int m,
                                       const float* const* wt_host, const float* const* bias_host, const float* const* f24_host,
                                       float* ind_out, void* stream);
int     buf_cost_volume_net_w24b(const float* s_eq, const float* t_eq, int m, const float* const* wt_host, const float* const* bias_host,
                                 const float* const* f24_host, float* ind_out, void* stream);
int     buf_cost_volume_net_w24b_gather(const float* equi, int ele_n, const long long* s_rows, const long long* t_rows, int m,
                                        const float* const* wt_host, const float* const* bias_host, const float* const* f24_host,
                                        float* ind_out, void* stream);

long long buf_split_gemm_count(int cout, int cin, int ntaps, int nt);
int     buf_split_tile_gemm(const float* w_host, int cout, int cin, int ntaps, int nt, unsigned short* out_host);
int     buf_cost_volume_net_split(const float* s_eq, const float* t_eq, int m, const void* const* wt_host,
                                  const float* const* bias_host, float* ind_out, int* status_dev, void* stream);
int     buf_cost_volume_net_split_gather(const float* equi, int ele_n, const long long* s_rows, const long long* t_rows, int m,
                                         const void* const* wt_host, const float* const* bias_host, float* ind_out,
                                         int* status_dev, void* stream);
int     buf_cost_volume_net_split_safe(const float* s_eq, const float* t_eq, int ele_n, const long long* s_rows, const long long* t_rows,
                                       int m, const void* const* wt_split_host, const float* const* bias_split_host,
                                       const float* const* wt_f32_host, const float* const* bias_f32_host, float* ind_out,
                                       int* status_dev, int* flags_ws, void* stream);
int     buf_cost_volume_net_split_safe_w24(const float* s_eq, const float* t_eq, int ele_n, const long long* s_rows, const long long* t_rows,
                                           int m, const void* const* wt_split_host, const float* const* bias_split_host,
                                           const float* const* wt_f32_host, const float* const* bias_f32_host, const float* const* f24_host,
                                           float* ind_out, int* status_dev, int* flags_ws, void* stream);
int     buf_cost_volume_net_split_safe_w24b(const float* s_eq, const float* t_eq, int ele_n, const long long* s_rows, const long long* t_rows,
                                            int m, const void* const* wt_split_host, const float* const* bias_split_host,
                                            const float* const* wt_f32_host, const float* const* bias_f32_host, const float* const* f24_host,
                                            float* ind_out, int* status_dev, int* flags_ws, void* stream);

int     buf_hypotheses_score(const float* ind, const float* ss_kpts, const float* tt_kpts, const float* ss_R,
                             const float* tt_R, int m, int azi_n, float inlier_th, float* R_out, float* t_out,
                             int* inlier_num, int* best_out, unsigned char* best_mask, void* stream);
size_t  buf_ransac_ws_bytes(int nhyp);
int     buf_ransac_kabsch(const float* src, const float* tgt, const int* corr, int ncorr, int nhyp,
                          unsigned long long seed, float max_dist, float edge_similarity, float* T_out,
                          int* info_out, void* ws, size_t ws_bytes, void* stream);
size_t  buf_ransac_masked_ws_bytes(int m, int nhyp);
int     buf_ransac_kabsch_masked(const float* src, const float* tgt, const unsigned char* mask, int m, int nhyp,
                                 unsigned long long seed, float max_dist, float edge_similarity, float* T_out,
                                 int* info_out, void* ws, size_t ws_bytes, void* stream);
int     buf_post_refine(const float* T_init, const float* src, const float* tgt, int m, float inlier_threshold,
                        int iters, float* T_out, int* info_out, void* stream);
size_t  buf_recover_poses_ws_bytes(int m_total, int nb, int nhyp);
int     buf_recover_poses_batched(const float* ind, const float* ss_kpts, const float* tt_kpts, const float* ss_R, const float* tt_R,
                                  const int* seg_host, int nb, const unsigned long long* seeds_host, int azi_n, float inlier_th,
                                  int nhyp, float max_dist, float edge_similarity, float refine_threshold, int refine_iters,
                                  float* poses_out, void* ws, size_t ws_bytes, void* stream);

size_t  buf_voxel_downsample_ws_bytes(int n, int64_t max_cells);
int     buf_voxel_downsample(const void* pts, const void* normals, int is_f64, int n, double voxel_size, double* out_pts,
                             double* out_normals, int* out_m_host, int64_t max_cells, void* ws, size_t ws_bytes, void* stream);
size_t  buf_voxel_downsample_batch_ws_bytes(int n, int nb, int64_t max_cells);
int     buf_voxel_downsample_batch(const void* pts, int is_f64, int n, const int* lengths_host, int nb, double voxel_size,
                                   double* out_pts, int* out_lengths_host, int64_t max_cells, void* ws, size_t ws_bytes, void* stream);
int     buf_knn_normals(const float* pts, int ns, const int* qidx, int nq, const int* cand, int ncand, int knn,
                        const double* camera_host, int orient, float* normals, unsigned char* deficient, void* stream);

#define BUF_ICP_POINT_TO_POINT 0
#define BUF_ICP_POINT_TO_PLANE 1
#define BUF_ICP_GENERALIZED 2
size_t  buf_icp_ws_bytes(int n_src_total, int n_tgt_total, int npairs, int method);
int     buf_icp_batched(const float* src, const int* src_lengths_host, const float* tgt, const float* tgt_normals,
                        const int* tgt_lengths_host, int npairs, int method, float max_dist, const double* T_init_f64,
                        int max_iteration, double rel_fitness, double rel_rmse, double* T_out_f64, double* fitness_out,
                        double* rmse_out, int* iters_out, int* nn_out, void* ws, size_t ws_bytes, void* stream);
int     buf_gicp_batched(const float* src, const float* src_normals, const int* src_lengths_host, const float* tgt,
                         const float* tgt_normals, const int* tgt_lengths_host, int npairs, float max_dist, double epsilon,
                         const double* T_init_f64, int max_iteration, double rel_fitness, double rel_rmse, double* T_out_f64,
                         double* fitness_out, double* rmse_out, int* iters_out, int* nn_out, void* ws, size_t ws_bytes, void* stream);

size_t  buf_fpfh_ws_bytes(int n);
int     buf_fpfh(const float* pts, const float* normals, int n, const int* nbr, int k_nbr, int max_nn,
                 double* fpfh_out , double* spfh_out ,
                 void* ws, size_t ws_bytes, void* stream);

int     buf_iss_keypoints(const float* pts, int n, const int* nbr_sal, int k_sal, const int* nbr_nms, int k_nms, int max_nn,
                          double gamma_21, double gamma_32, int min_neighbors, double* saliency_out ,
                          double* eig_out , unsigned char* mask_out , void* stream);

size_t  buf_feature_match_ws_bytes(long long na_total, long long nb_total, int pairs);
int     buf_feature_match(const float* fa, const int* a_lengths_host, const float* fb, const int* b_lengths_host,
                          int pairs, int d, int mutual, float ratio,
                          int* corr_out , int* counts_out ,
                          int* nn_out ,
                          float* ssd_out ,
                          void* ws, size_t ws_bytes, void* stream);

#define BUF_FGR_NOTHING 0
#define BUF_FGR_OK      1
#define BUF_FGR_FAILED  2
size_t  buf_fgr_ws_bytes(int n_corr_total, int npairs, int max_tuples);
int     buf_fgr_batched(const float* src, const int* src_lengths_host, const float* tgt, const int* tgt_lengths_host,
                        const int* corr ,
                        const int* corr_lengths_host, int npairs, const unsigned long long* seeds_host,
                        double tuple_scale, int max_tuples, int trial_factor,
                        double mu_start, double delta, int delta_absolute,
                        double division_factor, int decrease_every, int iterations,
                        double* T_out , int* info_out ,
                        int* rows_out , double* weights_out ,
                        void* ws, size_t ws_bytes, void* stream);

#define BUF_SC2_NOTHING 0
#define BUF_SC2_OK      1
#define BUF_SC2_MAX_ROWS 16384
size_t  buf_sc2_ws_bytes(const int* corr_lengths_host, int npairs, int max_seeds);
int     buf_sc2_batched(const float* src, const int* src_lengths_host, const float* tgt, const int* tgt_lengths_host,
                        const int* corr ,
                        const int* corr_lengths_host, int npairs,
                        double d_thr, double inlier_thr, double seed_ratio, int max_seeds,
                        int k1, double nms_radius, int power_iterations, int refine_iterations,
                        double* T_out , int* info_out ,
                        double* conf_out, int* seeds_out, int* hyp_counts_out, int* counts_out, unsigned char* inliers_out ,
                        void* ws, size_t ws_bytes, void* stream);

typedef struct buf_voxel_map {
    void*   buf;
    size_t  buf_bytes;
    int     nclouds, nrows, n;
    int64_t max_cells;
    double  voxel, epsilon;
    void*   clouds;
    int*    table;
    double* rows;
    long long* keys;
    int*    row_off;
} buf_voxel_map_t;
size_t  buf_voxel_map_bytes(int n_total, int nclouds, int64_t max_cells);
size_t  buf_voxel_map_ws_bytes(int n_total, int nclouds, int64_t max_cells);
int     buf_voxel_map_build(buf_voxel_map_t* map, const float* pts, const float* normals, const int* lengths_host, int nclouds,
                            double voxel, double epsilon, int64_t max_cells, void* buf, size_t buf_bytes, void* ws, size_t ws_bytes,
                            void* stream);
int     buf_voxel_map_export(const buf_voxel_map_t* map, int n, long long* keys, int* counts, double* means, double* covs,
                             int* row_off, void* stream);
size_t  buf_vgicp_ws_bytes(int n_src_total, int npairs);
int     buf_vgicp_batched(const buf_voxel_map_t* map, const float* src, const float* src_normals, const int* src_lengths_host,
                          const int* pair_cloud_host, int npairs, int neighbors, const double* T_init_f64, int max_iteration,
                          double rel_fitness, double rel_rmse, double* T_out_f64, double* fitness_out, double* rmse_out,
                          int* iters_out, int* row_out, void* ws, size_t ws_bytes, void* stream);

#define BUF_CLIQUE_NOTHING 0
#define BUF_CLIQUE_OK      1
size_t  buf_clique_ws_bytes(const int* corr_lengths_host, int npairs, int max_seeds, int max_members);
int     buf_clique_batched(const float* src, const int* src_lengths_host, const float* tgt, const int* tgt_lengths_host,
                           const int* corr ,
                           const int* corr_lengths_host, int npairs,
                           double d_thr, double tim_thr, double t_thr, double inlier_thr,
                           int max_seeds, int max_members, double gnc_factor, int gnc_iterations,
                           int refine_iterations,
                           double* T_out , int* info_out ,
                           int* deg_out, int* core_out, int* rank_out, int* sizes_out, int* members_out, double* weights_out,
                           double* pose0_out, unsigned char* inliers_out ,
                           void* ws, size_t ws_bytes, void* stream);

size_t  buf_pair_stats_ws_bytes(int n_total, int nclouds, int npairs, int n_src_rows, int64_t cells_per_elem);
int     buf_pair_stats(const float* pts, const int* lengths_host, int nclouds, const int* pair_src_host, const int* pair_tgt_host,
                       int npairs, const double* T_f64, float radius, int64_t cells_per_elem, int* matched_out,
                       double* moments_out, int* nn_out , void* ws, size_t ws_bytes, void* stream);

#define BUF_METRICS_NCOUNT     7
#define BUF_METRICS_REP_SRC    0
#define BUF_METRICS_REP_TGT    1
#define BUF_METRICS_NN_INL     2
#define BUF_METRICS_MUTUAL     3
#define BUF_METRICS_MUTUAL_INL 4
#define BUF_METRICS_CONS       5
#define BUF_METRICS_CONS_TRUE  6
int     buf_match_metrics(const float* kp, const int* s_nn, const int* t_nn, int npairs, int P, const double* T_gt_f64,
                          const float* T_est_f32, float tau_kp, float tau_match, float dist_th, int* out_counts,
                          float* out_nn_d2 , void* stream);

#define BUF_PG_MAX_NODES        128
#define BUF_PG_NOTHING          0
#define BUF_PG_CONVERGED_STEP   1
#define BUF_PG_CONVERGED_COST   2
#define BUF_PG_MAX_ITER         3
#define BUF_PG_STALLED          4
#define BUF_PG_FAILED           5
size_t  buf_pose_graph_ws_bytes(int ngraphs, int nodes_total, int edges_total, int max_nodes);
int     buf_pose_graph_optimize(const int* nodes_host, const int* edges_host, int ngraphs, const int* edge_i_host,
                                const int* edge_j_host, const double* Z_f64, const double* info_f64,
                                const unsigned char* uncertain_host, const int* fixed_host, const double* mu_host,
                                const double* X_init_f64, int max_iterations, double eps_step, double eps_cost, double tau0,
                                double* X_out_f64, int* status_out, double* cost_out, double* edge_out, void* ws, size_t ws_bytes,
                                void* stream);

#ifdef __cplusplus
}
#endif
#endif
```

Before: 179.0.

## Add row-6 tap-tiled direct convolution kernel and row-6-first ordering for 128-channel layers

Adds a new cylindrical-net kernel variant (w25t) for the 128-output-channel layers. It computes the boundary row 6 with a dedicated tap-tiled weight layout, loading weights as contiguous MFMA-ready tiles with software-prefetched loads. It can also run the row-6 direct pass before the Winograd pass, so the next weights can be primed while the direct pass finishes. Partial results are parked in AGPRs between passes, which trades register pressure for better load overlap. The path is selected by default through ROW6_DEFAULT='both' when no explicit forms are given, and it adds a separate host-side tiled tap array.

Measured after the change: 182.0 (median of 6 runs). +1.7%, better.

```diff
diff --git a/buffer_amd/_lib.py b/buffer_amd/_lib.py
--- a/buffer_amd/_lib.py
+++ b/buffer_amd/_lib.py
@@ -90,6 +90,9 @@
     "buf_cylindrical_net_w25_flags": (_i, [_vp, _vp, _vp, _vp, _vp]),
     "buf_cylindrical_net_split_safe_w25": (_i, [_vp, _i, _vp, _vp, _vp, _vp, _vp, _vp, _vp, _vp, _vp, _vp, _vp, _vp, _vp, _vp]),
     "buf_winograd_f25_tile_weights": (_i, [_vp, _i, _i, _vp]),
+    "buf_cylindrical_net_w25t": (_i, [_vp, _i, _vp, _vp, _vp, _vp, _vp, _vp, _vp, _vp, _i, _vp, _vp]),
+    "buf_cylindrical_net_split_safe_w25t": (_i, [_vp, _i, _vp, _vp, _vp, _vp, _vp, _vp, _vp, _vp, _vp, _i, _vp, _vp, _vp, _vp, _vp, _vp]),
+    "buf_cyl_row6_tile_taps": (_i, [_vp, _i, _i, _vp]),
     "buf_cylindrical_net_wg_supports": (_i, [_vp, _vp]),
     "buf_cylindrical_net_wg_flags": (_i, [_vp, _vp, _vp]),
     "buf_cylindrical_net_split_safe": (_i, [_vp, _i, _vp, _vp, _vp, _vp, _vp, _vp, _vp, _vp, _vp, _vp, _vp, _vp]),
diff --git a/buffer_amd/csrc/buffer_hip.hip b/buffer_amd/csrc/buffer_hip.hip
--- a/buffer_amd/csrc/buffer_hip.hip
+++ b/buffer_amd/csrc/buffer_hip.hip
@@ -20,6 +20,7 @@
 #include "convnet_w24p.hip"
 #include "convnet_w24a.hip"
 #include "convnet_w25.hip"
+#include "convnet_w25t.hip"
 #include "costnet.hip"
 #include "costnet_w24.hip"
 #include "costnet_w24b.hip"
diff --git a/buffer_amd/csrc/cnn_launch.hip b/buffer_amd/csrc/cnn_launch.hip
--- a/buffer_amd/csrc/cnn_launch.hip
+++ b/buffer_amd/csrc/cnn_launch.hip
@@ -8,10 +8,12 @@
 struct CylKernel { CylKernelFn plain, rerun; LdsGrant grant, grant_rerun; };
 static CylKernel cyl_wg = { k_cyl_net_wg, k_cyl_net_wg_rerun }, cyl_w24 = { k_cyl_net_w24, k_cyl_net_w24_rerun },
                  cyl_w24k = { k_cyl_net_w24k, k_cyl_net_w24k_rerun }, cyl_w24p = { k_cyl_net_w24p, k_cyl_net_w24p_rerun },
-                 cyl_w24a = { k_cyl_net_w24a, k_cyl_net_w24a_rerun }, cyl_w25 = { k_cyl_net_w25, k_cyl_net_w25_rerun };
-
-static CylKernel& cyl_kernel_for(const int* relu, int form, bool sets24, bool sets25)
-{
+                 cyl_w24a = { k_cyl_net_w24a, k_cyl_net_w24a_rerun }, cyl_w25 = { k_cyl_net_w25, k_cyl_net_w25_rerun },
+                 cyl_w25t = { k_cyl_net_w25t, k_cyl_net_w25t_rerun };
+
+static CylKernel& cyl_kernel_for(const int* relu, int form, bool sets24, bool sets25, bool taps)
+{
+    if (taps) return cyl_w25t;
     if (sets25) return cyl_w25;
     if (sets24) return cyl_w24a;
     bool flagged = false, ksplit = false;
@@ -58,8 +60,12 @@
     return BUF_OK;
 }
 
-static int cyl_check(const int* cin, const int* cout, const int* relu, const float* const* wt24_host, const float* const* wt25_host, const char* who)
-{
+static int cyl_check(const int* cin, const int* cout, const int* relu, const float* const* wt24_host, const float* const* wt25_host, const char* who,
+                     const float* const* taps_host = nullptr)
+{
+    for (int l = 0; taps_host && l < WG_LAYERS; l++)
+        BUF_REQUIRE(!taps_host[l] || cout[l] == 128, BUF_EINVAL, "%s: layer %d (%d -> %d) takes no row-6 tap set (128 output channels)", who, l,
+                    cin[l], cout[l]);
     if (!wt24_host && !wt25_host) {
         if (int rc = wg_check_widths(cin, cout)) return rc;
         for (int l = 0; l < WG_LAYERS; l++)
@@ -112,17 +118,19 @@
 }
 
 static int cyl_prepare(const float* const* wt_host, const float* const* bias_host, const int* cin_host, const int* cout_host, const int* relu_host,
-                       const float* const* wt24_host, const float* const* wt25_host, int form, const char* who, CylWgParams& P, CylKernel*& K)
+                       const float* const* wt24_host, const float* const* wt25_host, int form, const char* who, CylWgParams& P, CylKernel*& K,
+                       const float* const* taps_host = nullptr, int order = 0)
 {
     BUF_REQUIRE(wt_host && bias_host && cin_host && cout_host && relu_host, BUF_EINVAL, "%s: null argument", who);
     for (int l = 0; l < WG_LAYERS; l++) {
         P.wt[l] = wt_host[l]; P.bias[l] = bias_host[l];
         P.cin[l] = cin_host[l]; P.cout[l] = cout_host[l]; P.relu[l] = relu_host[l];
+        P.taps[l] = nullptr;
         BUF_REQUIRE(P.wt[l] && P.bias[l], BUF_EINVAL, "%s: null weights for layer %d", who, l);
     }
-    if (int rc = cyl_check(P.cin, P.cout, P.relu, wt24_host, wt25_host, who)) return rc;
+    if (int rc = cyl_check(P.cin, P.cout, P.relu, wt24_host, wt25_host, who, taps_host)) return rc;
     P.only_if = nullptr;
-    K = &cyl_kernel_for(P.relu, form, wt24_host != nullptr, wt25_host != nullptr);
+    K = &cyl_kernel_for(P.relu, form, wt24_host != nullptr, wt25_host != nullptr, taps_host != nullptr);
     if (K == &cyl_wg) return BUF_OK;
     for (int l = 0; l < WG_LAYERS; l++) {
         if (wt25_host && wt25_host[l]) { P.wt[l] = wt25_host[l]; P.relu[l] = (P.relu[l] & 1) | W25_FLAG; }
@@ -130,6 +138,10 @@
         else if (P.relu[l] & W24K_FLAG) P.wt[l] += WG_BLOCKS * P.cout[l] * P.cin[l];
         else if (wt24_host && wt24_host[l]) { P.wt[l] = wt24_host[l]; P.relu[l] |= W24K_FLAG; }
         P.relu[l] &= ~WG_F24_FLAG;
+        if (taps_host && P.cout[l] == 128) {
+            if (taps_host[l]) { P.taps[l] = taps_host[l]; P.relu[l] |= W25T_TAPS; }
+            if (order & BUF_CYL_ROW6_FIRST) P.relu[l] |= W25T_FIRST;
+        }
     }
     return BUF_OK;
 }
@@ -207,14 +219,15 @@
 
 static int cyl_net_own_sets(const char* who, const float* x, int npatch, const float* const* wt_host, const float* const* bias_host, const int* cin_host,
                             const int* cout_host, const int* relu_host, const float* const* wt24_host, const float* const* wt25_host, bool w25, float* y,
-                            void* stream)
+                            void* stream, bool w25t = false, const float* const* taps_host = nullptr, int order = 0)
 {
     BUF_REQUIRE(npatch >= 0, BUF_EINVAL, "%s: npatch=%d", who, npatch);
+    BUF_REQUIRE(!w25t || (order & ~BUF_CYL_ROW6_FIRST) == 0, BUF_EINVAL, "%s: order=%d (0, or BUF_CYL_ROW6_FIRST = 1)", who, order);
     if (npatch == 0) return BUF_OK;
-    BUF_REQUIRE(x && y && wt24_host && (wt25_host || !w25), BUF_EINVAL, "%s: null argument", who);
+    BUF_REQUIRE(x && y && wt24_host && (wt25_host || !w25) && (taps_host || !w25t), BUF_EINVAL, "%s: null argument", who);
     CylWgParams P;
     CylKernel* K;
-    if (int rc = cyl_prepare(wt_host, bias_host, cin_host, cout_host, relu_host, wt24_host, wt25_host, BUF_CYL_FORM_DEFAULT, who, P, K)) return rc;
+    if (int rc = cyl_prepare(wt_host, bias_host, cin_host, cout_host, relu_host, wt24_host, wt25_host, BUF_CYL_FORM_DEFAULT, who, P, K, taps_host, order)) return rc;
     return cyl_launch(*K, x, npatch, P, y, stream);
 }
 
@@ -229,6 +242,14 @@
                                        void* stream)
 {
     return cyl_net_own_sets("buf_cylindrical_net_w25", x, npatch, wt_host, bias_host, cin_host, cout_host, relu_host, wt24_host, wt25_host, true, y, stream);
+}
+
+extern "C" int buf_cylindrical_net_w25t(const float* x, int npatch, const float* const* wt_host, const float* const* bias_host, const int* cin_host,
+                                        const int* cout_host, const int* relu_host, const float* const* wt24_host, const float* const* wt25_host,
+                                        const float* const* taps_host, int order, float* y, void* stream)
+{
+    return cyl_net_own_sets("buf_cylindrical_net_w25t", x, npatch, wt_host, bias_host, cin_host, cout_host, relu_host, wt24_host, wt25_host, true, y, stream,
+                            true, taps_host, order);
 }
 
 template <typename Q>
diff --git a/buffer_amd/csrc/convnet_w25t.hip b/buffer_amd/csrc/convnet_w25t.hip
--- /dev/null
+++ b/buffer_amd/csrc/convnet_w25t.hip
@@ -0,0 +1,224 @@
+#include "common.h"
+
+#define W25T_TAPS 16
+#define W25T_FIRST 32
+#define W25T_STRIDE 768
+
+#define W25T_G(n, k, a, b) T[k][((n) * 6 + (a) * 3 + (b)) >> 2][((n) * 6 + (a) * 3 + (b)) & 3]
+
+template <bool PRIME>
+__device__ __forceinline__ void w25t_round_direct(unsigned row5, __amdgpu_buffer_rsrc_t rt, unsigned tp, unsigned lofs4, int niter,
+                                                  const float* __restrict__ bias_lane, wgf4 (&Y)[2], __amdgpu_buffer_rsrc_t rs, unsigned wp,
+                                                  unsigned lofs2, wgf4 (&W4)[2][2], wgf2 (&W2)[2][2])
+{
+    wgf4 T[2][3];
+#pragma unroll
+    for (int k = 0; k < 2; k++)
+#pragma unroll
+        for (int q = 0; q < 3; q++) T[k][q] = wg_ldw(rt, tp + k * W25T_STRIDE + q * 256, lofs4);
+    float X[2][6];
+    unsigned pa = row5;
+    WG_LOADD(X[0], pa, 0)
+    WG_LOADD(X[1], pa, WG_KSTEP)
+    wgf4 acc[2][3];
+    float zero = 0.f;
+    asm volatile("" : "+v"(zero));
+#pragma unroll
+    for (int n = 0; n < 2; n++) {
+        acc[n][0] = (wgf4){ zero, zero, zero, zero };
+        acc[n][1] = (wgf4){ zero, zero, zero, zero };
+        acc[n][2] = *reinterpret_cast<const wgf4*>(bias_lane + n * 16);
+    }
+    auto iteration = [&](auto last, unsigned tcur) __attribute__((always_inline)) {
+        constexpr bool LAST = decltype(last)::value;
+        __builtin_amdgcn_sched_barrier(0);
+#pragma unroll
+        for (int s = 0; s < 4; s++) {
+#pragma unroll
+            for (int b = 0; b < 3; b++)
+#pragma unroll
+                for (int a = 0; a < 2; a++)
+#pragma unroll
+                    for (int n = 0; n < 2; n++)
+                        acc[n][b] = __builtin_amdgcn_mfma_f32_16x16x4f32(W25T_G(n, s & 1, a, b), X[s & 1][a * 3 + b], acc[n][b], 0, 0, 0);
+            __builtin_amdgcn_sched_barrier(0);
+            if (s < 2) WG_LOADD(X[s & 1], pa, (s + 2) * WG_KSTEP)
+            else if constexpr (!LAST) {
+                if (s == 2) {
+                    pa += 4u * WG_KSTEP;
+                    asm volatile("" : "+v"(pa));
+                }
+                WG_LOADD(X[s & 1], pa, (s - 2) * WG_KSTEP)
+            }
+            __builtin_amdgcn_sched_barrier(0);
+            if (s < 2 || !LAST) {
+#pragma unroll
+                for (int q = 0; q < 3; q++) T[s & 1][q] = wg_ldw(rt, tcur + (s + 2) * W25T_STRIDE + q * 256, lofs4);
+            } else if constexpr (PRIME) {
+#pragma unroll
+                for (int n = 0; n < 2; n++) {
+                    W4[n][s & 1] = wg_ldw(rs, wp + (s & 1) * W24_WSTRIDE + n * 256, lofs4);
+                    W2[n][s & 1] = w24_ldw2(rs, wp + (s & 1) * W24_WSTRIDE + 512 + n * 128, lofs2);
+                }
+            }
+            __builtin_amdgcn_sched_barrier(0);
+        }
+    };
+#pragma unroll 1
+    for (int it = 0; it < niter - 1; it++) iteration(std::false_type{}, tp + 4 * it * W25T_STRIDE);
+    iteration(std::true_type{}, tp + 4 * (niter - 1) * W25T_STRIDE);
+#pragma unroll
+    for (int n = 0; n < 2; n++) Y[n] = (acc[n][0] + acc[n][1]) + acc[n][2];
+}
+
+template <bool TAPS, bool FIRST>
+__device__ __forceinline__ void w25t_layer_pair(float* __restrict__ act, const float* __restrict__ wt, const float* __restrict__ taps,
+                                                const float* __restrict__ bias, int cin, int relu, int pair, const WgAddrPark& pk,
+                                                const W24AddrPark& pk24)
+{
+    static_assert(TAPS || FIRST, "neither: w24_layer_pair");
+    act[(threadIdx.x >> 1) * WG_CS + WG_ZERO + 4 + (threadIdx.x & 1)] = 0.f;
+    __syncthreads();
+    int lane = threadIdx.x & (WAVE - 1);
+    asm volatile("" : "+v"(lane));
+    const int lk = lane >> 4;
+    const int k4 = cin >> 2;
+    const __amdgpu_buffer_rsrc_t rs = wg_weights(wt);
+    const __amdgpu_buffer_rsrc_t rt = wg_weights(TAPS ? taps : wt);
+    const unsigned pstride = (unsigned)(k4 * W24_WSTRIDE);
+    const unsigned wp = (unsigned)pair * 4 * pstride;
+    const unsigned tp = (unsigned)(pair * k4) * W25T_STRIDE;
+    const unsigned lofs4 = lane * 16, lofs2 = lane * 8;
+    const float* bv = bias + (2 * pair) * 16 + lk * 4;
+    wgf4 W4[2][2];
+    wgf2 W2[2][2];
+    wgf4 Y[2][2][4];
+    wgf4 Yb[2];
+    float park[2][36];
+    auto first_steps = [&](bool narrow) __attribute__((always_inline)) {
+#pragma unroll
+        for (int n = 0; n < 2; n++)
+#pragma unroll
+            for (int k = 0; k < 2; k++) {
+                W4[n][k] = wg_ldw(rs, wp + k * W24_WSTRIDE + n * 256, lofs4);
+                if (narrow) W2[n][k] = w24_ldw2(rs, wp + k * W24_WSTRIDE + 512 + n * 128, lofs2);
+            }
+    };
+    auto park_row6 = [&]() __attribute__((always_inline)) {
+#pragma unroll
+        for (int n = 0; n < 2; n++)
+#pragma unroll
+            for (int q = 0; q < 4; q++) asm volatile("v_accvgpr_write_b32 %0, %1" : "=a"(park[n][32 + q]) : "v"(Yb[n][q]));
+    };
+    auto winograd = [&]() __attribute__((always_inline)) {
+        unsigned RA[4];
+#pragma unroll
+        for (int a = 0; a < 4; a++) asm volatile("v_accvgpr_read_b32 %0, %1" : "=v"(RA[a]) : "a"(pk24.a[a]));
+        w24_round(RA, rs, wp, wp, lofs4, lofs2, k4 >> 2, pstride, bv, W4, W2, Y);
+    };
+    const unsigned row5 = wg_parked(pk, 2, 0);
+    if constexpr (FIRST) {
+        if constexpr (TAPS) w25t_round_direct<true>(row5, rt, tp, lofs4, k4 >> 2, bv, Yb, rs, wp, lofs2, W4, W2);
+        else {
+            first_steps(false);
+            w24_round_direct(row5, rs, wp, lofs4, k4 >> 2, pstride, bv, W4, Yb);
+        }
+        park_row6();
+        if constexpr (!TAPS) first_steps(true);
+        winograd();
+    } else {
+        first_steps(true);
+        winograd();
+#pragma unroll
+        for (int n = 0; n < 2; n++)
+#pragma unroll
+            for (int q = 0; q < 32; q++) asm volatile("v_accvgpr_write_b32 %0, %1" : "=a"(park[n][q]) : "v"(Y[n][q >> 4][(q >> 2) & 3][q & 3]));
+        w25t_round_direct<false>(row5, rt, tp, lofs4, k4 >> 2, bv, Yb, rs, wp, lofs2, W4, W2);
+        park_row6();
+    }
+    __syncthreads();
+    int lane_s = threadIdx.x & (WAVE - 1);
+    asm volatile("" : "+v"(lane_s));
+#pragma unroll
+    for (int n = 0; n < 2; n++) {
+        if constexpr (!FIRST) {
+#pragma unroll
+            for (int q = 0; q < 32; q++) asm volatile("v_accvgpr_read_b32 %0, %1" : "=v"(Y[n][q >> 4][(q >> 2) & 3][q & 3]) : "a"(park[n][q]));
+        }
+#pragma unroll
+        for (int q = 0; q < 4; q++) asm volatile("v_accvgpr_read_b32 %0, %1" : "=v"(Yb[n][q]) : "a"(park[n][32 + q]));
+        w24_store_tile(Y[n], 2 * pair + n, relu, act, lane_s & 15, lane_s >> 4);
+        wg_store_row6<false>(Yb[n], 2 * pair + n, relu, act, nullptr, lane_s & 15, lane_s >> 4);
+    }
+}
+
+__device__ __forceinline__ void cyl_net_w25t_body(const float* __restrict__ x, const CylWgParams& P, float* __restrict__ y, float* __restrict__ lds)
+{
+    float* act = lds;
+    const int patch = blockIdx.x;
+    const int w0 = __builtin_amdgcn_readfirstlane(threadIdx.x / WAVE);
+    wg_load_input(x, P, act, patch);
+    WgAddrPark pk;
+    W24AddrPark pk24;
+    {
+        int lane0 = threadIdx.x & (WAVE - 1);
+        asm volatile("" : "+v"(lane0));
+        wg_park_addresses(act, lane0 & 15, lane0 >> 4, pk);
+        w24_park_addresses(act, lane0 & 15, lane0 >> 4, pk24);
+    }
+#pragma unroll 1
+    for (int l = 0; l < WG_LAYERS; l++) {
+        int w = w0;
+        asm volatile("" : "+s"(w));
+        const int cin = P.cin[l], cout = P.cout[l], relu = P.relu[l] & 1;
+        const bool f24 = (P.relu[l] & W24K_FLAG) != 0, f25 = (P.relu[l] & W25_FLAG) != 0;
+        const bool tp = (P.relu[l] & W25T_TAPS) != 0, df = (P.relu[l] & W25T_FIRST) != 0;
+        float* yp = y + (size_t)patch * cout * 140;
+        if (f25 && cout == 64) w25_layer_psplit<4, false>(act, nullptr, P.wt[l], P.bias[l], cin, relu, w);
+        else if (f25 && l < WG_LAYERS - 1) w25_layer_psplit<2, false>(act, nullptr, P.wt[l], P.bias[l], cin, relu, w);
+        else if (f25) w25_layer_psplit<2, true>(act, yp, P.wt[l], P.bias[l], cin, relu, w);
+        else if (cout == 128 && tp && df) w25t_layer_pair<true, true>(act, P.wt[l], P.taps[l], P.bias[l], cin, relu, w0, pk, pk24);
+        else if (cout == 128 && tp) w25t_layer_pair<true, false>(act, P.wt[l], P.taps[l], P.bias[l], cin, relu, w0, pk, pk24);
+        else if (cout == 128 && df) w25t_layer_pair<false, true>(act, P.wt[l], nullptr, P.bias[l], cin, relu, w0, pk, pk24);
+        else if (cout == 128) w24_layer_pair(act, P.wt[l], P.bias[l], cin, relu, w0, pk, pk24);
+        else if (cout == 64 && f24) w24p_layer_psplit(act, P.wt[l], P.bias[l], cin, relu, w, pk, pk24);
+        else if (cout == 64) wg_layer_msplit(act, P.wt[l], P.bias[l], cin, cout, relu, w, pk);
+        else if (f24 && l < WG_LAYERS - 1) w24a_layer_psplit32<false>(act, nullptr, P.wt[l], P.bias[l], cin, relu, w, pk, pk24);
+        else if (f24) w24a_layer_psplit32<true>(act, yp, P.wt[l], P.bias[l], cin, relu, w, pk, pk24);
+        else if (l < WG_LAYERS - 1) wg_layer_mksplit<false>(act, nullptr, P.wt[l], P.bias[l], cin, cout, relu, w, pk);
+        else wg_layer_mksplit<true>(act, yp, P.wt[l], P.bias[l], cin, cout, relu, w, pk);
+        __syncthreads();
+    }
+}
+
+__global__ void __launch_bounds__(WG_THREADS, 2) k_cyl_net_w25t(const float* __restrict__ x, CylWgParams P, float* __restrict__ y)
+{
+    extern __shared__ float lds[];
+    cyl_net_w25t_body(x, P, y, lds);
+}
+
+__global__ void __launch_bounds__(WG_THREADS, 2) k_cyl_net_w25t_rerun(const float* __restrict__ x, CylWgParams P, float* __restrict__ y)
+{
+    extern __shared__ float lds[];
+    if (P.only_if[blockIdx.x] == 0) return;
+    cyl_net_w25t_body(x, P, y, lds);
+}
+
+extern "C" int buf_cyl_row6_tile_taps(const float* w_host, int cout, int cin, float* out_host)
+{
+    BUF_REQUIRE(w_host && out_host, BUF_EINVAL, "buf_cyl_row6_tile_taps: null argument");
+    BUF_REQUIRE(cout > 0 && cin > 0 && cout % 32 == 0 && cin % 4 == 0, BUF_EINVAL, "buf_cyl_row6_tile_taps: widths %d -> %d", cin, cout);
+    const int k4 = cin / 4;
+    for (int o = 0; o < cout; o++)
+        for (int c = 0; c < cin; c++) {
+            const float* g = w_host + ((size_t)o * cin + c) * 9;
+            const int n = o / 16, lane = (c % 4) * 16 + o % 16;
+            float* blk = out_host + ((size_t)(n / 2) * k4 + c / 4) * W25T_STRIDE;
+            for (int a = 0; a < 2; a++)
+                for (int b = 0; b < 3; b++) {
+                    const int f = 6 * (n % 2) + 3 * a + b;
+                    blk[(f / 4) * 256 + lane * 4 + f % 4] = g[3 * a + b];
+                }
+        }
+    return BUF_OK;
+}
diff --git a/buffer_amd/csrc/convnet_wg.hip b/buffer_amd/csrc/convnet_wg.hip
--- a/buffer_amd/csrc/convnet_wg.hip
+++ b/buffer_amd/csrc/convnet_wg.hip
@@ -20,6 +20,7 @@
     const float* bias[WG_LAYERS];
     int cin[WG_LAYERS], cout[WG_LAYERS], relu[WG_LAYERS];
     const int* only_if;
+    const float* taps[WG_LAYERS];
 #ifdef WG_STAMP
     long long* stamps;
 #endif
diff --git a/buffer_amd/csrc/split_safe.hip b/buffer_amd/csrc/split_safe.hip
--- a/buffer_amd/csrc/split_safe.hip
+++ b/buffer_amd/csrc/split_safe.hip
@@ -53,16 +53,19 @@
 static int cyl_split_safe_own_sets(const char* who, const char* who_f32, const float* x, int npatch, const void* const* wt_split_host,
                                    const float* const* wt_wg_host, const float* const* bias_host, const int* cin_host, const int* cout_host,
                                    const int* relu_host, const float* const* wt24_host, const float* const* wt25_host, bool w25, const float* head_params,
-                                   float* y_or_equi, float* desc, int* status_dev, int* flags_ws, void* stream)
+                                   float* y_or_equi, float* desc, int* status_dev, int* flags_ws, void* stream, bool w25t = false,
+                                   const float* const* taps_host = nullptr, int order = 0)
 {
     BUF_REQUIRE(npatch >= 0, BUF_EINVAL, "%s: npatch=%d", who, npatch);
+    BUF_REQUIRE(!w25t || (order & ~BUF_CYL_ROW6_FIRST) == 0, BUF_EINVAL, "%s: order=%d (0, or BUF_CYL_ROW6_FIRST = 1)", who, order);
     if (npatch == 0) return BUF_OK;
     BUF_REQUIRE(x && y_or_equi && flags_ws && wt_split_host, BUF_EINVAL, "%s: null argument", who);
     BUF_REQUIRE(!head_params || desc, BUF_EINVAL, "%s: head without desc", who);
-    BUF_REQUIRE(wt24_host && (wt25_host || !w25), BUF_EINVAL, "%s: null argument", who_f32);
+    BUF_REQUIRE(wt24_host && (wt25_host || !w25) && (taps_host || !w25t), BUF_EINVAL, "%s: null argument", who_f32);
     CylWgParams P;
     CylKernel* K;
-    if (int rc = cyl_prepare(wt_wg_host, bias_host, cin_host, cout_host, relu_host, wt24_host, wt25_host, BUF_CYL_FORM_DEFAULT, who_f32, P, K)) return rc;
+    if (int rc = cyl_prepare(wt_wg_host, bias_host, cin_host, cout_host, relu_host, wt24_host, wt25_host, BUF_CYL_FORM_DEFAULT, who_f32, P, K, taps_host, order))
+        return rc;
     return cyl_split_safe(x, npatch, wt_split_host, bias_host, cin_host, cout_host, relu_host, *K, P, head_params, y_or_equi, desc, status_dev, flags_ws, stream);
 }
 
@@ -82,6 +85,17 @@
 {
     return cyl_split_safe_own_sets("buf_cylindrical_net_split_safe_w25", "buf_cylindrical_net_w25", x, npatch, wt_split_host, wt_wg_host, bias_host,
                                    cin_host, cout_host, relu_host, wt24_host, wt25_host, true, head_params, y_or_equi, desc, status_dev, flags_ws, stream);
+}
+
+extern "C" int buf_cylindrical_net_split_safe_w25t(const float* x, int npatch, const void* const* wt_split_host, const float* const* wt_wg_host,
+                                                   const float* const* bias_host, const int* cin_host, const int* cout_host, const int* relu_host,
+                                                   const float* const* wt24_host, const float* const* wt25_host, const float* const* taps_host,
+                                                   int order, const float* head_params, float* y_or_equi, float* desc, int* status_dev,
+                                                   int* flags_ws, void* stream)
+{
+    return cyl_split_safe_own_sets("buf_cylindrical_net_split_safe_w25t", "buf_cylindrical_net_w25t", x, npatch, wt_split_host, wt_wg_host, bias_host,
+                                   cin_host, cout_host, relu_host, wt24_host, wt25_host, true, head_params, y_or_equi, desc, status_dev, flags_ws, stream,
+                                   true, taps_host, order);
 }
 
 template <typename Q>
diff --git a/buffer_amd/ops.py b/buffer_amd/ops.py
--- a/buffer_amd/ops.py
+++ b/buffer_amd/ops.py
@@ -990,6 +990,31 @@
     return sets, (C.c_void_p * len(sets))(*[None if t is None else t.data_ptr() for t in sets])
 
 
+ROW6_DEFAULT = 'both'
+ROW6_PARTS = {'both': (True, True), 'all': (True, True), 'taps': (True, False), 'order': (False, True), 'off': (False, False), None: (False, False)}
+
+
+def cyl_row6_tile_taps(w):
+    cout, cin = w.shape[0], w.shape[1]
+    assert cin % 4 == 0 and cout % 32 == 0
+    t = np.asarray(w, np.float32)[:, :, :2, :].reshape(cout // 32, 2, 16, cin // 4, 4, 6)
+    t = np.transpose(t, (0, 3, 4, 2, 1, 5)).reshape(cout // 32, cin // 4, 4, 16, 3, 4)
+    return np.ascontiguousarray(np.transpose(t, (0, 1, 4, 2, 3, 5))).reshape(-1)
+
+
+def cyl_row6_parts(f24, f24k, f24p, row6, f24a=None, f25=None):
+    explicit = not (f24 is None and f24k is None and f24p is None and f24a is None and f25 is None)
+    parts = form_parts('row6', row6, None if explicit else ROW6_DEFAULT, ROW6_PARTS)
+    if any(parts) and not (f24 in (None, True) and f24k in (None, True) and f24p in (None, True)):
+        raise ValueError("row6 goes with the default forms of the other layers (f24, f24k, f24p left alone or true)")
+    return parts
+
+
+def cyl_row6_taps(layers, flags, taps, device):
+    sets = [torch.from_numpy(cyl_row6_tile_taps(w)).to(device) if (taps and flag == F24_FLAG) else None for (w, _, _), flag in zip(layers, flags)]
+    return sets, (C.c_void_p * len(sets))(*[None if t is None else t.data_ptr() for t in sets])
+
+
 def cyl_layer_filters(w, f24k=True):
     wt = winograd_tile_weights(w)
     cout, cin = w.shape[0], w.shape[1]
@@ -1020,8 +1045,9 @@
 
 class CylindricalNet:
 
-    def __init__(self, layers, device, f24=None, f24k=None, f24p=None, f24a=None, f25=None):
+    def __init__(self, layers, device, f24=None, f24k=None, f24p=None, f24a=None, f25=None, row6=None):
         parts25 = cyl_f25_parts(f24, f24k, f24p, f25)
+        row6_taps, row6_first = cyl_row6_parts(f24, f24k, f24p, row6, f24a, f25)
         f24, f24k, f24p, parts = cyl_f24a_parts(f24, f24k, f24p, f24a)
         self.wt, self.bias, self.cin, self.cout, self.relu = [], [], [], [], []
         self.entry = "buf_cylindrical_net_wg"
@@ -1045,7 +1071,12 @@
         self.f24_all = bool(self.f24_layers) and all(f or t is not None for f, t in zip(flags, self.wt24))
         self.wt25, self._w25p = cyl_f25_filters(layers, parts25, device)
         self.f25_layers = [l for l, t in enumerate(self.wt25) if t is not None]
-        if self.f25_layers:
+        self.taps, self._tapsp = cyl_row6_taps(layers, flags, row6_taps, device)
+        self.taps_layers = [l for l, t in enumerate(self.taps) if t is not None]
+        self.row6_first = bool(row6_first and F24_FLAG in flags)
+        if self.taps_layers or self.row6_first:
+            fn, safe, self._extra = "w25t", "split_safe_w25t", (self._w24p, self._w25p, self._tapsp, 1 if self.row6_first else 0)
+        elif self.f25_layers:
             fn, safe, self._extra = "w25", "split_safe_w25", (self._w24p, self._w25p)
         elif self.f24_layers:
             fn, safe, self._extra = "wg_all", "split_safe_all", (self._w24p,)
@@ -1072,12 +1103,13 @@
 
 class CylindricalNetSplit:
 
-    def __init__(self, layers, device, f24k=None, f24p=None, f24a=None, f25=None):
+    def __init__(self, layers, device, f24k=None, f24p=None, f24a=None, f25=None, row6=None):
         cyl_f25_parts(None, f24k, f24p, f25)
+        cyl_row6_parts(None, f24k, f24p, row6, f24a, f25)
         form = cyl_f24a_parts(None, f24k, f24p, f24a)[2]
         self.wt, self.bias, self.cin, self.cout, self.relu = [], [], [], [], []
         self.entry = "buf_cylindrical_net_split"
-        self.f24_layers, self.f24_all, self.f25_layers = [], False, []
+        self.f24_layers, self.f24_all, self.f25_layers, self.taps_layers, self.row6_first = [], False, [], [], False
         self.form = 1 if form else 0
         for w, b, relu in layers:
             cout, cin = w.shape[0], w.shape[1]
@@ -1093,12 +1125,13 @@
         self._re = (C.c_int * n)(*self.relu)
         self.last_flags = None
         self.safe = n == 8 and _lib.lib().buf_cylindrical_net_wg_supports(self._ci, self._co) == 0 and not os.environ.get('BUF_SPLIT_UNSAFE')
-        self.f32 = CylindricalNet(layers, device, f24k=f24k, f24p=f24p, f24a=f24a, f25=f25) if self.safe else None
+        self.f32 = CylindricalNet(layers, device, f24k=f24k, f24p=f24p, f24a=f24a, f25=f25, row6=row6) if self.safe else None
         if self.safe:
             f = self.f32
             self.wt_wg, self._wwp, self._re_safe = f.wt, f._wp, f._re
             self.wt24, self._w24p, self.f24_layers, self.f24_all = f.wt24, f._w24p, f.f24_layers, f.f24_all
             self.wt25, self._w25p, self.f25_layers = f.wt25, f._w25p, f.f25_layers
+            self.taps, self._tapsp, self.taps_layers, self.row6_first = f.taps, f._tapsp, f.taps_layers, f.row6_first
             self.fn = f.fn_split_safe
 
     def _safe_call(self, x, head):
diff --git a/include/buffer_hip.h b/include/buffer_hip.h
--- a/include/buffer_hip.h
+++ b/include/buffer_hip.h
@@ -170,6 +170,11 @@
 int     buf_cylindrical_net_w25(const float* x, int npatch, const float* const* wt_host, const float* const* bias_host,
                                 const int* cin_host, const int* cout_host, const int* relu_host, const float* const* wt24_host,
                                 const float* const* wt25_host, float* y, void* stream);
+#define BUF_CYL_ROW6_FIRST 1
+int     buf_cyl_row6_tile_taps(const float* w_host, int cout, int cin, float* out_host);
+int     buf_cylindrical_net_w25t(const float* x, int npatch, const float* const* wt_host, const float* const* bias_host,
+                                 const int* cin_host, const int* cout_host, const int* relu_host, const float* const* wt24_host,
+                                 const float* const* wt25_host, const float* const* taps_host, int order, float* y, void* stream);
 
 long long buf_split_filter_count(int cout, int cin);
 int     buf_split_tile_filters(const float* w_host, int cout, int cin, unsigned short* out_host);
@@ -195,6 +200,11 @@
                                            const float* const* bias_host, const int* cin_host, const int* cout_host, const int* relu_host,
                                            const float* const* wt24_host, const float* const* wt25_host, const float* head_params,
                                            float* y_or_equi, float* desc, int* status_dev, int* flags_ws, void* stream);
+int     buf_cylindrical_net_split_safe_w25t(const float* x, int npatch, const void* const* wt_split_host, const float* const* wt_wg_host,
+                                            const float* const* bias_host, const int* cin_host, const int* cout_host, const int* relu_host,
+                                            const float* const* wt24_host, const float* const* wt25_host, const float* const* taps_host,
+                                            int order, const float* head_params, float* y_or_equi, float* desc, int* status_dev,
+                                            int* flags_ws, void* stream);
 
 int     buf_descriptor_head(const float* y, int npatch, const float* params, float* desc, float* equi, void* stream);
 
```
